# VachaLab/gorder

Measured on AMD Instinct MI355X. Metric: trajectory frames/sec, higher is better.
Workload: dtype f32

## Files before the change

### gorder_amd/abi.py

```python
from __future__ import annotations

import ctypes as C
import os
from dataclasses import dataclass, field
from typing import List, Optional, Sequence

import numpy as np

_HERE = os.path.dirname(os.path.abspath(__file__))
LIB_PATH = os.environ.get("GORDER_HIP_LIB") or os.path.join(_HERE, "libgorder_hip.so")

OK = 0
ERR_UNDEFINED_BOX = 1
ERR_NOT_ORTHOGONAL_BOX = 2
ERR_ZERO_BOX = 3
ERR_UNDEFINED_POSITION = 4
ERR_INVALID_GLOBAL_MEMBRANE_CENTER = 5
ERR_INVALID_LOCAL_MEMBRANE_CENTER = 6
ERR_INVALID_ARGUMENT = 100
ERR_DEVICE = 101
ERR_NO_DEVICE = 102
ERR_BOX_RANGE = 103
ERR_LEAFLETS_NOT_PRIMED = 104
ERR_OVERFLOW = 105
# ... 119 lines not shown
    flip: bool = False
    radius: float = 0.0
    membrane: Optional[np.ndarray] = None


@dataclass
class OrderMap:
    enabled: bool = False
    plane: int = 0
    span_x: Sequence[float] = (0.0, 0.0)
    span_y: Sequence[float] = (0.0, 0.0)
    bin: Sequence[float] = (0.1, 0.1)


GEOM_NONE, GEOM_CUBOID, GEOM_CYLINDER, GEOM_SPHERE = range(4)
GEOMREF_POINT, GEOMREF_BOX_CENTER, GEOMREF_GROUP = range(3)
_INF = float("inf")


@dataclass
class Geometry:
    kind: int = GEOM_NONE
    invert: bool = False
    reference: int = GEOMREF_POINT
    point: Sequence[float] = (0.0, 0.0, 0.0)
    group: Optional[np.ndarray] = None
    xdim: Sequence[float] = (-_INF, _INF)
    ydim: Sequence[float] = (-_INF, _INF)
    zdim: Sequence[float] = (-_INF, _INF)
    radius: float = 0.0
    span: Sequence[float] = (-_INF, _INF)
    orientation: int = 2
    structure_box: Sequence[float] = (0.0, 0.0, 0.0)


@dataclass
class DynamicNormal:
    enabled: bool = False
    radius: float = 2.0
    cloud: Optional[np.ndarray] = None


@dataclass
class Tables:
    n_atoms: int
    molecule_types: List[MolType]
    handle_pbc: bool = True
    normal: Sequence[float] = (0.0, 0.0, 1.0)
    leaflets: Leaflets = field(default_factory=Leaflets)
    ordermap: OrderMap = field(default_factory=OrderMap)
    timewise: bool = False
    device: int = 0
    flags: int = 0
    geometry: Geometry = field(default_factory=Geometry)
    dynamic_normal: DynamicNormal = field(default_factory=DynamicNormal)

    @property
    def n_acc(self) -> int:
        return sum(m.n_slots for m in self.molecule_types)

    @property
    def n_molecules_total(self) -> int:
        return sum(m.n_molecules for m in self.molecule_types)

    @property
    def n_samples_per_frame(self) -> int:
        return sum(m.n_slots * m.n_molecules for m in self.molecule_types)

    def as_ctypes(self):
        keep = []
        mts = (CMolType * max(1, len(self.molecule_types)))()
        for k, m in enumerate(self.molecule_types):
            c = mts[k]
            c.n_molecules = m.n_molecules
            b = _u32(m.bonds, (-1, m.n_molecules, 2)) if m.bonds is not None else None
            c.n_bond_types = 0 if b is None else b.shape[0]
            c.bonds = _ptr(b)
            ua = (CUaAtom * max(1, len(m.ua_atoms)))()
            for q, (kind, idx) in enumerate(m.ua_atoms):
                ia = _u32(idx, (m.n_molecules, 4))
                ua[q].kind = int(kind)
                ua[q].indices = _ptr(ia)
                keep.append(ia)
            c.n_ua_atoms = len(m.ua_atoms)
            c.ua_atoms = C.cast(ua, C.POINTER(CUaAtom))
            h = _u32(m.heads, (m.n_molecules,)) if m.heads is not None else None
            c.heads = _ptr(h)
            me = _u32(m.methyls, (m.n_molecules, -1)) if m.methyls is not None else None
            c.n_methyls = 0 if me is None else me.shape[1]
            c.methyls = _ptr(me)
            nh = _u32(m.normal_heads, (m.n_molecules,)) if m.normal_heads is not None else None
            c.normal_heads = _ptr(nh)
            keep += [b, ua, h, me, nh]
        t = CTables()
        t.n_atoms = self.n_atoms
        t.n_molecule_types = len(self.molecule_types)
        t.molecule_types = C.cast(mts, C.POINTER(CMolType))
        t.handle_pbc = 1 if self.handle_pbc else 0
        t.normal[:] = [float(x) for x in self.normal]
        lf = self.leaflets
        mem = _u32(lf.membrane) if lf.membrane is not None else None
        t.leaflets.method = lf.method
        t.leaflets.normal_dim = lf.normal_dim
        t.leaflets.frequency = lf.frequency
        t.leaflets.flip = 1 if lf.flip else 0
        t.leaflets.radius = lf.radius
        t.leaflets.n_membrane = 0 if mem is None else mem.size
        t.leaflets.membrane = _ptr(mem)
        om = self.ordermap
        t.ordermap.enabled = 1 if om.enabled else 0
        t.ordermap.plane = om.plane
        t.ordermap.span_x[:] = [float(x) for x in om.span_x]
        t.ordermap.span_y[:] = [float(x) for x in om.span_y]
        t.ordermap.bin[:] = [float(x) for x in om.bin]
        t.timewise = 1 if self.timewise else 0
        t.device = self.device
        t.flags = self.flags
        ge = self.geometry
        grp = _u32(ge.group) if ge.group is not None else None
        t.geometry.kind = ge.kind
        t.geometry.invert = 1 if ge.invert else 0
        t.geometry.reference = ge.reference
        t.geometry.point[:] = [float(x) for x in ge.point]
        t.geometry.n_group = 0 if grp is None else grp.size
        t.geometry.group = _ptr(grp)
        t.geometry.xdim[:] = [float(x) for x in ge.xdim]
        t.geometry.ydim[:] = [float(x) for x in ge.ydim]
        t.geometry.zdim[:] = [float(x) for x in ge.zdim]
        t.geometry.radius = ge.radius
        t.geometry.span[:] = [float(x) for x in ge.span]
        t.geometry.orientation = ge.orientation
        t.geometry.structure_box[:] = [float(x) for x in ge.structure_box]
        dn = self.dynamic_normal
        cloud = _u32(dn.cloud) if dn.cloud is not None else None
        t.dynamic_normal.enabled = 1 if dn.enabled else 0
        t.dynamic_normal.radius = dn.radius
        t.dynamic_normal.n_cloud = 0 if cloud is None else cloud.size
        t.dynamic_normal.cloud = _ptr(cloud)
        keep += [mts, mem, grp, cloud]
        return t, keep


_EXPORTS = [
    "gorder_hip_create", "gorder_hip_destroy", "gorder_hip_n_accumulators", "gorder_hip_ordermap_dims",
    "gorder_hip_set_stream", "gorder_hip_submit_device", "gorder_hip_submit_host",
    "gorder_hip_prime_leaflets", "gorder_hip_set_manual_leaflets", "gorder_hip_synchronize",
    "gorder_hip_finish", "gorder_hip_timewise", "gorder_hip_leaflets", "gorder_hip_leaflet_distances",
    "gorder_hip_normals", "gorder_hip_export_maps", "gorder_hip_set_normals",
    "gorder_hip_accumulators_device", "gorder_hip_bind_accumulators", "gorder_hip_last_error_index", "gorder_hip_last_error_frame", "gorder_hip_kernel_time_names",
    "gorder_hip_last_error_message", "gorder_hip_strerror", "gorder_hip_kernel_time", "gorder_hip_kernel_time_group", "gorder_hip_plan",
    "gorder_hip_plan_tables", "gorder_hip_selftest_arithmetic", "gorder_hip_selftest_trig", "gorder_hip_run_trajectory",
    "gorder_hip_comm_unique_id", "gorder_hip_comm_create", "gorder_hip_comm_destroy", "gorder_hip_allreduce",
    "gorder_hip_reset", "gorder_hip_xtc_decode", "gorder_hip_release_staging", "gorder_hip_speculation_stats", "gorder_hip_local_decide_stats",
    "gorder_hip_spherical_stats",
]

_lib = None


class GorderHipError(RuntimeError):
    def __init__(self, status: int, message: str = "", index: int = 0, frame: int = 0):
        self.status = status
        self.index = index
        self.frame = frame
        super().__init__(f"gorder_hip status {status}: {message}")


def load_library() -> C.CDLL:
    global _lib
    if _lib is not None:
        return _lib
    if not os.path.exists(LIB_PATH):
        raise GorderHipError(ERR_NO_DEVICE, f"{LIB_PATH} is missing: run `python -c 'import __graft_entry__ as g; "
                                            "g.build()'` (there is no CPU fallback)")
    try:
        import torch
        _rt = os.path.join(os.path.dirname(torch.__file__), "lib", "libamdhip64.so")
        if os.path.exists(_rt):
            C.CDLL(_rt, mode=C.RTLD_GLOBAL)
    except ImportError:
        pass
    lib = C.CDLL(LIB_PATH)
    vp, u32, u64, i32 = C.c_void_p, C.c_uint32, C.c_uint64, C.c_int
    lib.gorder_hip_create.argtypes = [C.POINTER(CTables), C.POINTER(vp)]
    lib.gorder_hip_destroy.argtypes = [vp]
    lib.gorder_hip_destroy.restype = None
    lib.gorder_hip_n_accumulators.argtypes = [vp]
    lib.gorder_hip_n_accumulators.restype = u32
    lib.gorder_hip_ordermap_dims.argtypes = [vp, C.POINTER(u32), C.POINTER(u32)]
    lib.gorder_hip_ordermap_dims.restype = u32
    lib.gorder_hip_set_stream.argtypes = [vp, vp]
    lib.gorder_hip_submit_device.argtypes = [vp, vp, vp, vp, u32]
    lib.gorder_hip_submit_host.argtypes = [vp, vp, vp, vp, u32]
    lib.gorder_hip_prime_leaflets.argtypes = [vp, vp, vp, u64]
    lib.gorder_hip_set_manual_leaflets.argtypes = [vp, vp, u64]
    lib.gorder_hip_synchronize.argtypes = [vp]
    lib.gorder_hip_finish.argtypes = [vp, vp, vp, vp, vp, C.POINTER(u64)]
    lib.gorder_hip_timewise.argtypes = [vp, vp, vp, u64]
    lib.gorder_hip_leaflets.argtypes = [vp, vp, C.POINTER(u64)]
    lib.gorder_hip_leaflet_distances.argtypes = [vp, vp]
    lib.gorder_hip_normals.argtypes = [vp, vp, vp]
    lib.gorder_hip_export_maps.argtypes = [vp, vp, vp, u64]
    lib.gorder_hip_set_normals.argtypes = [vp, vp, u32]
    lib.gorder_hip_accumulators_device.argtypes = [vp, C.POINTER(vp), C.POINTER(u64)]
    lib.gorder_hip_bind_accumulators.argtypes = [vp, vp, u64]
    lib.gorder_hip_last_error_index.argtypes = [vp]
    lib.gorder_hip_last_error_index.restype = u64
    lib.gorder_hip_kernel_time_names.argtypes = [vp]
    lib.gorder_hip_kernel_time_names.restype = C.c_char_p
    lib.gorder_hip_last_error_frame.argtypes = [vp]
    lib.gorder_hip_last_error_frame.restype = u64
    lib.gorder_hip_last_error_message.argtypes = [vp]
    lib.gorder_hip_last_error_message.restype = C.c_char_p
    lib.gorder_hip_strerror.argtypes = [i32]
    lib.gorder_hip_strerror.restype = C.c_char_p
    lib.gorder_hip_kernel_time.argtypes = [vp, C.POINTER(C.c_double), C.POINTER(u64), i32]
    lib.gorder_hip_kernel_time_group.argtypes = [vp, C.c_uint32, C.POINTER(C.c_char_p), C.POINTER(C.c_double), C.POINTER(u64)]
    lib.gorder_hip_plan.argtypes = [vp, C.POINTER(CPlan)]
    lib.gorder_hip_speculation_stats.argtypes = [vp, C.POINTER(C.c_uint64)]
    lib.gorder_hip_local_decide_stats.argtypes = [vp, C.POINTER(C.c_uint64)]
    lib.gorder_hip_spherical_stats.argtypes = [vp, C.POINTER(C.c_float)]
    lib.gorder_hip_plan_tables.argtypes = [C.POINTER(CTables), C.POINTER(CPlan), C.POINTER(i32)]
    lib.gorder_hip_selftest_arithmetic.argtypes = [i32, C.c_uint64, C.c_uint64, C.POINTER(C.c_uint64)]
    lib.gorder_hip_selftest_trig.argtypes = [i32, i32, C.c_uint32, C.c_uint32, C.c_uint32, C.c_void_p]
    lib.gorder_hip_run_trajectory.argtypes = [vp, C.POINTER(CTrajectory), C.POINTER(CTrajectoryStats)]
    lib.gorder_hip_comm_unique_id.argtypes = [vp]
    lib.gorder_hip_comm_create.argtypes = [vp, vp, i32, i32, C.POINTER(vp)]
    lib.gorder_hip_comm_destroy.argtypes = [vp]
    lib.gorder_hip_comm_destroy.restype = None
    lib.gorder_hip_allreduce.argtypes = [vp, vp]
    lib.gorder_hip_reset.argtypes = [vp]
    lib.gorder_hip_xtc_decode.argtypes = [vp, vp, u64, vp, u32, u32, vp, u32, vp, u32]
    lib.gorder_hip_release_staging.argtypes = [vp]
    lib.gorder_hip_release_staging.restype = None
    _lib = lib
    return lib


def selftest_trig(fn: str, first_bits: int, stride: int, n: int, device: int = 0) -> np.ndarray:
    lib = load_library()
    out = np.empty(n, dtype=np.float32)
    st = lib.gorder_hip_selftest_trig(device, {"acos": 0, "acos_cores": 1, "cos": 2, "sin": 3}[fn], first_bits, stride, n, out.ctypes.data)
    if st != 0:
        raise GorderHipError(st, "gorder_hip_selftest_trig")
    return out


def selftest_arithmetic(n: int = 1 << 26, seed: int = 1, device: int = 0):
    lib = load_library()
    out = (C.c_uint64 * 2)()
    st = lib.gorder_hip_selftest_arithmetic(device, n, seed, out)
    if st != 0:
        raise GorderHipError(st, lib.gorder_hip_strerror(st).decode())
    return int(out[0]), int(out[1])


def plan_tables(tables: Tables) -> dict:
    lib = load_library()
    ct, keep = tables.as_ctypes()
    plan, check = CPlan(), C.c_int(-1)
    st = lib.gorder_hip_plan_tables(C.byref(ct), C.byref(plan), C.byref(check))
    if st != OK:
        raise GorderHipError(st, lib.gorder_hip_strerror(st).decode())
    d = {name: getattr(plan, name) for name, _ in CPlan._fields_}
    d["selfcheck"] = check.value
    return d


@dataclass
class Results:
    sums: np.ndarray
    counts: np.ndarray
    n_frames: int
    map_sums: Optional[np.ndarray] = None
    map_counts: Optional[np.ndarray] = None

    def order_ticks(self, min_samples: int = 1) -> np.ndarray:
        n = self.counts.astype(np.int64)
        ok = n >= max(1, min_samples)
        q = np.full(self.sums.shape, np.iinfo(np.int64).min, dtype=np.int64)
        q[ok] = (np.abs(self.sums[ok]) // n[ok]) * np.sign(self.sums[ok])
        return q

    def order(self, min_samples: int = 1) -> np.ndarray:
        out = np.full(self.sums.shape, np.nan, dtype=np.float32)
        n = self.counts.astype(np.int64)
        ok = n >= max(1, min_samples)
        q = (np.abs(self.sums[ok]) // n[ok]) * np.sign(self.sums[ok])
        out[ok] = (q.astype(np.float64) / 1e6).astype(np.float32)
        return out


class HipEngine:

    def __init__(self, tables: Tables):
        self.lib = load_library()
        self.tables = tables
        ct, keep = tables.as_ctypes()
        self._h = C.c_void_p()
        st = self.lib.gorder_hip_create(C.byref(ct), C.byref(self._h))
        if st != OK:
            msg = self.lib.gorder_hip_strerror(st).decode()
            if self._h:
                msg += ": " + self.lib.gorder_hip_last_error_message(self._h).decode()
                self.lib.gorder_hip_destroy(self._h)
                self._h = C.c_void_p()
            raise GorderHipError(st, msg)
        self.n_acc = self.lib.gorder_hip_n_accumulators(self._h)
        self._keep = []

    def close(self):
        if getattr(self, "_h", None):
            self.lib.gorder_hip_destroy(self._h)
            self._h = C.c_void_p()

    def __del__(self):
        try:
            self.close()
        except Exception:
            pass

    def _check(self, st: int):
        if st != OK:
            msg = self.lib.gorder_hip_strerror(st).decode() + ": " + \
                self.lib.gorder_hip_last_error_message(self._h).decode()
            raise GorderHipError(st, msg, self.lib.gorder_hip_last_error_index(self._h),
                                 self.lib.gorder_hip_last_error_frame(self._h))

    def set_stream(self, stream_ptr: int):
        self._check(self.lib.gorder_hip_set_stream(self._h, C.c_void_p(stream_ptr)))

    def use_torch_stream(self):
        import torch
        self.set_stream(torch.cuda.current_stream().cuda_stream)

    @staticmethod
    def _frame_index(frame_index, n_frames):
        if frame_index is None:
            frame_index = np.arange(n_frames, dtype=np.uint64)
        fi = np.ascontiguousarray(frame_index, dtype=np.uint64)
        assert fi.shape == (n_frames,)
        return fi

    def submit_device(self, xyz, box, frame_index=None):
        assert xyz.is_cuda and xyz.is_contiguous() and xyz.dtype.is_floating_point and xyz.element_size() == 4
        n_frames = xyz.shape[0]
        assert xyz.shape[1] == self.tables.n_atoms and xyz.shape[2] == 3
        fi = self._frame_index(frame_index, n_frames)
        bp = None
        if box is not None:
            assert box.is_cuda and box.is_contiguous() and box.numel() == 9 * n_frames
            bp = C.c_void_p(box.data_ptr())
        self._check(self.lib.gorder_hip_submit_device(self._h, C.c_void_p(xyz.data_ptr()), bp,
                                                      fi.ctypes.data_as(C.c_void_p), n_frames))

    def submit_host(self, xyz: np.ndarray, box: Optional[np.ndarray], frame_index=None):
        xyz = np.ascontiguousarray(xyz, dtype=np.float32)
        n_frames = xyz.shape[0]
        assert xyz.shape[1:] == (self.tables.n_atoms, 3)
        fi = self._frame_index(frame_index, n_frames)
        bp = None
        if box is not None:
            box = np.ascontiguousarray(box, dtype=np.float32).reshape(n_frames, 9)
            bp = box.ctypes.data_as(C.c_void_p)
        self._check(self.lib.gorder_hip_submit_host(self._h, xyz.ctypes.data_as(C.c_void_p), bp,
                                                    fi.ctypes.data_as(C.c_void_p), n_frames))

    def run_trajectory(self, paths, group=None, begin: float = 0.0, end: float = -1.0, step: int = 1, threads: int = 0,
                       batch_frames: int = 0, first_frame_index: int = 0, device_decode: bool = False,
                       shard=None) -> dict:
        arr = (C.c_char_p * len(paths))(*[p.encode() for p in paths])
        grp = None if group is None else np.ascontiguousarray(group, dtype=np.uint32)
        t = CTrajectory()
# ... 4 lines not shown
        t.begin_ps, t.end_ps, t.step = begin, end, step
        t.n_threads, t.batch_frames, t.first_frame_index = threads, batch_frames, first_frame_index
        t.device_decode = 1 if device_decode else 0
        if shard is not None:
            t.shard_index, t.shard_count = shard
        stats = CTrajectoryStats()
        self._check(self.lib.gorder_hip_run_trajectory(self._h, C.byref(t), C.byref(stats)))
        return {name: getattr(stats, name) for name, _ in CTrajectoryStats._fields_}

    def xtc_decode(self, d_blob: int, blob_bytes: int, d_frames: int, n_frames: int, n_atoms_file: int, d_slot_of: int,
                   n_stop: int, d_xyz: int, n_atoms_out: int):
        self._check(self.lib.gorder_hip_xtc_decode(self._h, d_blob, blob_bytes, d_frames, n_frames, n_atoms_file,
                                                   d_slot_of or None, n_stop, d_xyz, n_atoms_out))

    def release_staging(self):
        self.lib.gorder_hip_release_staging(self._h)

    def reset(self):
        self._check(self.lib.gorder_hip_reset(self._h))

    @staticmethod
    def comm_unique_id() -> bytes:
        lib = load_library()
        buf = (C.c_uint8 * 128)()
        st = lib.gorder_hip_comm_unique_id(buf)
        if st != OK:
            raise GorderHipError(st, "ncclGetUniqueId failed (is RCCL loadable?)")
        return bytes(buf)

    def comm_create(self, unique_id: bytes, n_ranks: int, rank: int):
        assert len(unique_id) == 128
        buf = (C.c_uint8 * 128).from_buffer_copy(unique_id)
        comm = C.c_void_p()
        self._check(self.lib.gorder_hip_comm_create(self._h, buf, n_ranks, rank, C.byref(comm)))
        return comm

    def comm_destroy(self, comm):
        self.lib.gorder_hip_comm_destroy(comm)

    def allreduce(self, comm):
        self._check(self.lib.gorder_hip_allreduce(self._h, comm))

    def prime_leaflets_device(self, xyz, box, frame_index: int):
        bp = C.c_void_p(box.data_ptr()) if box is not None else None
        self._check(self.lib.gorder_hip_prime_leaflets(self._h, C.c_void_p(xyz.data_ptr()), bp, frame_index))

    def set_manual_leaflets(self, flags: np.ndarray, frame_index: int = 0):
        flags = np.ascontiguousarray(flags, dtype=np.uint8)
        assert flags.size == self.tables.n_molecules_total
        self._check(self.lib.gorder_hip_set_manual_leaflets(self._h, flags.ctypes.data_as(C.c_void_p), frame_index))

    def synchronize(self):
        self._check(self.lib.gorder_hip_synchronize(self._h))

    def ordermap_dims(self):
        nx, ny = C.c_uint32(), C.c_uint32()
        nt = self.lib.gorder_hip_ordermap_dims(self._h, C.byref(nx), C.byref(ny))
        return (int(nx.value), int(ny.value)) if nt else (0, 0)

    def finish(self) -> Results:
        n = self.n_acc
        sums = np.zeros((3, n), dtype=np.int64)
        counts = np.zeros((3, n), dtype=np.uint64)
        nx, ny = C.c_uint32(), C.c_uint32()
        nt = self.lib.gorder_hip_ordermap_dims(self._h, C.byref(nx), C.byref(ny))
        ms = mc = None
        msp = mcp = None
        if nt:
            ms = np.zeros((3, n, nx.value, ny.value), dtype=np.int64)
            mc = np.zeros((3, n, nx.value, ny.value), dtype=np.uint64)
            msp, mcp = ms.ctypes.data_as(C.c_void_p), mc.ctypes.data_as(C.c_void_p)
        nf = C.c_uint64()
        self._check(self.lib.gorder_hip_finish(self._h, sums.ctypes.data_as(C.c_void_p),
                                               counts.ctypes.data_as(C.c_void_p), msp, mcp, C.byref(nf)))
        return Results(sums, counts, int(nf.value), ms, mc)

    def timewise(self, n_frames: int):
        n = self.n_acc
        s = np.zeros((n_frames, 3, n), dtype=np.int64)
        c = np.zeros((n_frames, 3, n), dtype=np.uint64)
        self._check(self.lib.gorder_hip_timewise(self._h, s.ctypes.data_as(C.c_void_p),
                                                 c.ctypes.data_as(C.c_void_p), n_frames))
        return s, c

    def leaflets(self):
        flags = np.zeros(self.tables.n_molecules_total, dtype=np.uint8)
        fr = C.c_uint64()
        self._check(self.lib.gorder_hip_leaflets(self._h, flags.ctypes.data_as(C.c_void_p), C.byref(fr)))
        return flags, int(fr.value)

    def leaflet_distances(self) -> np.ndarray:
        d = np.zeros(self.tables.n_molecules_total, dtype=np.float32)
        self._check(self.lib.gorder_hip_leaflet_distances(self._h, d.ctypes.data_as(C.c_void_p)))
        return d

    def set_normals(self, normals: np.ndarray):
        n = np.ascontiguousarray(normals, dtype=np.float32)
        assert n.ndim == 3 and n.shape[1:] == (self.tables.n_molecules_total, 3)
        self._check(self.lib.gorder_hip_set_normals(self._h, n.ctypes.data_as(C.c_void_p), n.shape[0]))

    def normals(self):
        n = np.zeros((self.tables.n_molecules_total, 3), dtype=np.float32)
        k = np.zeros(self.tables.n_molecules_total, dtype=np.uint32)
        self._check(self.lib.gorder_hip_normals(self._h, n.ctypes.data_as(C.c_void_p), k.ctypes.data_as(C.c_void_p)))
        return n, k

    def accumulator_words(self) -> int:
        p, n = C.c_void_p(), C.c_uint64()
        self._check(self.lib.gorder_hip_accumulators_device(self._h, C.byref(p), C.byref(n)))
        return int(n.value)

    def flush(self):
        self.accumulator_words()

    def bind_accumulators(self, tensor):
        assert tensor.is_cuda and tensor.is_contiguous() and tensor.element_size() == 8
        self._keep.append(tensor)
        self._check(self.lib.gorder_hip_bind_accumulators(self._h, C.c_void_p(tensor.data_ptr()), tensor.numel()))

    def export_maps(self, sums, counts):
        for t in (sums, counts):
            assert t.is_cuda and t.is_contiguous() and t.element_size() == 8
        assert sums.numel() == counts.numel()
        self._check(self.lib.gorder_hip_export_maps(self._h, C.c_void_p(sums.data_ptr()), C.c_void_p(counts.data_ptr()),
                                                     sums.numel()))

    def kernel_time(self, reset: bool = False):
        ms, n = C.c_double(), C.c_uint64()
        self._check(self.lib.gorder_hip_kernel_time(self._h, C.byref(ms), C.byref(n), 1 if reset else 0))
        return ms.value, int(n.value)

    def kernel_names(self) -> str:
        return self.lib.gorder_hip_kernel_time_names(self._h).decode()

    def kernel_groups(self):
        out, k = [], 0
        while True:
            name, ms, n = C.c_char_p(), C.c_double(), C.c_uint64()
            if self.lib.gorder_hip_kernel_time_group(self._h, k, C.byref(name), C.byref(ms), C.byref(n)) != 0:
                return out
            out.append((name.value.decode(), ms.value, int(n.value)))
            k += 1

    def speculation_stats(self) -> dict:
        out = (C.c_uint64 * 4)()
        self._check(self.lib.gorder_hip_speculation_stats(self._h, out))
        return {"batches": int(out[0]), "moved": int(out[1]), "exact_frames": int(out[2]), "enabled": bool(out[3])}

    def local_decide_stats(self) -> dict:
        out = (C.c_uint64 * 4)()
        self._check(self.lib.gorder_hip_local_decide_stats(self._h, out))
        return {"submits": int(out[0]), "paused": int(out[1]), "open_frames": int(out[2]), "frames": int(out[3])}

    def spherical_stats(self) -> dict:
        out = (C.c_float * 12)()
        self._check(self.lib.gorder_hip_spherical_stats(self._h, out))
        v = np.array(out[:], dtype=np.float32)
        return {"centre": v[0:3].copy(), "weight_a": v[3], "mean_a": v[4], "var_a": v[5], "mean_b": v[6], "var_b": v[7],
                "avg_log_likelihood": v[8], "iterations": int(v[9]), "n_outer": int(v[10])}

    def plan(self) -> dict:
        p = CPlan()
        self._check(self.lib.gorder_hip_plan(self._h, C.byref(p)))
        return {name: getattr(p, name) for name, _ in CPlan._fields_}
```

### gorder_amd/csrc/gorder_hip.hip

```cpp
#include <hip/hip_runtime.h>

#include <dlfcn.h>

#include <cmath>
#include <cstdio>
#include <cstdlib>
#include <cstring>
#include <mutex>
#include <new>
#include <string>
#include <deque>
#include <vector>

#include "../../include/gorder_hip.h"
#include "gm_math.h"
#include "plan.h"

#pragma clang fp contract(off)

using gorder::DirectItem;
using gorder::Item;
using gorder::kBlock;
using gorder::Plan;
using gorder::Tile;

#include "kernels_common.h"
#include "kernels_bonds.h"
#include "kernels_extras.h"
#include "kernels_leaflets.h"
#include "kernels_normals.h"
#include "kernels_xtc.h"


struct gorder_hip_handle {
    void *traj_cache = nullptr;
    void (*traj_cache_free)(gorder_hip_handle *) = nullptr;
    Plan plan;
    gorder_tables_t tables{};
    int device = 0;
    hipStream_t own_stream = nullptr;
    hipStream_t stream = nullptr;
    Tile *d_tiles = nullptr;
    Item *d_items = nullptr;
    uint32_t *d_tile_slots = nullptr;
    DirectItem *d_direct = nullptr;
    Tile *d_ua_tiles = nullptr;
    gorder::UaItem *d_ua_items = nullptr;
    uint32_t *d_ua_tile_slots = nullptr;
    uint32_t map_nx = 0, map_ny = 0;
    unsigned long long *d_map_sums = nullptr, *d_map_cnts = nullptr;
    unsigned long long *d_map_packed = nullptr;
    unsigned long long *d_map_rec = nullptr;
    size_t map_rec_cap = 0;
    gorder::MapRun *d_ua_runs = nullptr, *d_runs = nullptr;
    uint32_t *d_ua_run_begin = nullptr, *d_run_begin = nullptr;
    Item *d_items_by_slot = nullptr;
    uint32_t *d_ua_item_run = nullptr, *d_item_run = nullptr;
    uint4 *d_lgrid = nullptr;
    LocalRowPre *d_lrowpre = nullptr;
    LocalEdge *d_ledge = nullptr;
    float4 *d_lfinfo = nullptr;
    static constexpr uint32_t kDecidePause = 16;
    uint32_t *d_lsummary = nullptr, *h_lsummary = nullptr;
    hipEvent_t lsummary_written = nullptr;
    bool lsummary_pending = false;
    uint32_t decide_pause = 0;
    uint64_t decide_submits = 0, decide_paused_submits = 0;
    uint32_t *d_lneed = nullptr;
    uint2 *d_ltodo = nullptr;
    size_t map_lds_bytes = 0;
    bool map_staged = false;
    uint64_t map_pending = 0;
    uint64_t map_fold_limit = kMapFoldLimit;
    uint32_t map_max_mol = 1;
    unsigned long long *d_tw_sums = nullptr, *d_tw_cnts = nullptr;
    uint64_t tw_cap = 0;
    ExtraArgs extra{};
    uint32_t *d_geom_group = nullptr;
    float *d_shapes = nullptr;
    float *d_inv_box = nullptr;
    size_t inv_box_cap = 0;
    uint32_t dyn_slab = 4, local_slab = 4;
    bool local_halo = false;
    size_t local_rec_stride = 0;
    XtcCheckpoint *d_xtc_cp = nullptr;
    size_t xtc_cp_cap = 0;
    bool dyn = false;
    uint32_t *d_dyn_cloud = nullptr, *d_dyn_heads = nullptr;
    uint32_t *d_dyn_cell_of = nullptr, *d_dyn_count = nullptr;
    float *d_dyn_rec = nullptr;
    float4 *d_dyn_normals = nullptr;
    DynCov *d_dyn_cov = nullptr;
    size_t dyn_normals_cap = 0;
    std::vector<float> last_normals;
    std::vector<float> manual_normals;
    uint32_t manual_frames = 0;
    bool manual_active = false;
    size_t shapes_cap = 0;
    uint32_t *d_err = nullptr;
    unsigned long long *d_acc = nullptr;
    unsigned long long *d_rep = nullptr;
    uint32_t n_rep = 32;
    bool rep_dirty = false;
    bool acc_external = false;
    size_t acc_words = 0;
    uint32_t *d_heads = nullptr, *d_membrane = nullptr, *d_methyl_begin = nullptr, *d_methyl_atoms = nullptr;
    uint8_t *d_aflags = nullptr;
    size_t aflags_rows = 0;
    float *d_adist = nullptr;
    float *d_sph_spill = nullptr, *d_sph_stats = nullptr;
    uint32_t sph_spill = 0, sph_slab = 1u << 20, sph_threads = 1024;
    uint32_t *d_lcell_of = nullptr, *d_lcell_count = nullptr, *d_lcell_fill = nullptr;
    float *d_ltrig = nullptr;
    uint32_t *d_arow = nullptr, *d_aframes = nullptr;
    std::vector<uint32_t> up_arow, up_aframes;
    const uint32_t *up_arow_at = nullptr, *up_aframes_at = nullptr;
    size_t arow_cap = 0, aframes_cap = 0;
    bool have_assignment = false;
    uint64_t assignment_frame = 0;
    bool spec_enabled = false;
    bool spec_now = false;
    uint2 *d_own = nullptr;
    float4 *d_mom = nullptr;
    size_t mom_cap = 0;
    float *d_head_z = nullptr;
    size_t head_z_cap = 0;
    uint32_t *d_own_head_begin = nullptr;
    uint2 *d_own_heads = nullptr;
    float *d_spec_center = nullptr;
    uint8_t *d_spec_ok = nullptr;
    size_t spec_frames_cap = 0;
    uint32_t *d_spec_counters = nullptr;
    static constexpr uint32_t kSpecRing = 8;
    uint32_t *h_spec_counters = nullptr;
    hipEvent_t spec_counters_copied[kSpecRing] = {};
    uint64_t spec_ring_frames[kSpecRing] = {};
    uint32_t *d_spec_mol_begin = nullptr;
    SpecSample *d_spec_samples = nullptr;
    uint64_t spec_batches = 0, spec_fixed = 0, spec_exact_frames = 0;
    float *d_stage_xyz[2] = {nullptr, nullptr}, *d_stage_box[2] = {nullptr, nullptr};
    size_t stage_xyz_cap[2] = {0, 0}, stage_box_cap[2] = {0, 0};
    hipEvent_t stage_copied[2] = {nullptr, nullptr}, stage_computed[2] = {nullptr, nullptr};
    bool stage_used[2] = {false, false};
    int stage_next = 0;
    hipStream_t copy_stream = nullptr;
    float n2 = 1.0f, n2sq = 1.0f;
    int axis = -1;
    int frames_per_stage = kFramesPerStage;
    bool membrane_is_frame = false;
    bool use_gather = false;
    uint32_t wg_capacity = 256u * 6u;
    uint32_t wg_target = 0;
    uint32_t lw = 0;
    size_t lds_bytes = 0;
    uint64_t n_frames = 0;
    uint64_t err_index = 0;
    std::string err_msg;
    static constexpr uint32_t kTimingEvents = 1024;
    struct TimingSeg { uint32_t label, ev_a, ev_b; };
    bool timing_on = false;
    hipEvent_t timing_ev[kTimingEvents] = {};
    uint32_t timing_next_ev = 0;
    int timing_open_label = -1;
    uint32_t timing_open_ev = 0;
    std::deque<TimingSeg> timing_pending;
    std::vector<std::string> timing_labels;
    std::vector<double> timing_label_ms;
    std::vector<uint64_t> timing_label_n;
    uint64_t timing_launches = 0;
    std::string timed_kernels;
    std::vector<uint32_t> host_heads, host_dyn_heads;
    uint32_t *d_mol_slot0 = nullptr;
    uint64_t err_frame = 0;
    struct BatchLog { uint64_t ordinal, first, stride; std::vector<uint64_t> list; };
    static constexpr size_t kBatchLog = 4096;
    std::deque<BatchLog> batch_log;
    uint64_t n_submits = 0;
    const unsigned long long *decoder_key = nullptr;
};

namespace {

int fail(gorder_hip_handle *h, int status, const std::string &msg) {
    if (h) h->err_msg = msg;
    return status;
}

#define HIP_TRY(h, expr)                                                                    \
    do {                                                                                    \
        hipError_t e_ = (expr);                                                             \
        if (e_ != hipSuccess)                                                               \
            return fail(h, GORDER_ERR_DEVICE, std::string(#expr) + ": " + hipGetErrorString(e_)); \
    } while (0)

template <typename T>
int upload(gorder_hip_handle *h, T **dst, const std::vector<T> &src) {
    *dst = nullptr;
    if (src.empty()) return GORDER_OK;
    HIP_TRY(h, hipMalloc((void **)dst, src.size() * sizeof(T)));
    HIP_TRY(h, hipMemcpy(*dst, src.data(), src.size() * sizeof(T), hipMemcpyHostToDevice));
    return GORDER_OK;
}

template <typename T>
int ensure(gorder_hip_handle *h, T **buf, size_t *cap, size_t need) {
    if (need <= *cap) return GORDER_OK;
    if (*buf) HIP_TRY(h, hipFree(*buf));
    *buf = nullptr;
    *cap = 0;
    const size_t n = need + need / 2;
    HIP_TRY(h, hipMalloc((void **)buf, n * sizeof(T)));
    *cap = n;
    return GORDER_OK;
}

bool should_assign(uint32_t frequency, uint64_t frame) {
// ... 773 lines not shown
        if (e != hipSuccess || per_cu < 1) per_cu = 4;
        h->wg_capacity = (uint32_t)n_cu * (uint32_t)per_cu;
    }

    const gorder_dynamic_normal_t &dn = t->dynamic_normal;
    if (dn.enabled) {
        if (!(dn.radius > 0.0f)) return fail(h, GORDER_ERR_INVALID_ARGUMENT, "dynamic normals need a positive radius");
        if (!dn.cloud || dn.n_cloud == 0) return fail(h, GORDER_ERR_INVALID_ARGUMENT, "dynamic normals need the NormalHeads group");
        if (!p.direct.empty()) return fail(h, GORDER_ERR_INVALID_ARGUMENT, "dynamic normals: a bond spans more than the LDS window");
        std::vector<uint32_t> cloud(dn.cloud, dn.cloud + dn.n_cloud), nheads;
        for (uint32_t a : cloud)
            if (a >= t->n_atoms) return fail(h, GORDER_ERR_INVALID_ARGUMENT, "NormalHeads index out of range");
        for (uint32_t m = 0; m < t->n_molecule_types; m++) {
            const gorder_moltype_t &mt = t->molecule_types[m];
            if (!mt.normal_heads) return fail(h, GORDER_ERR_INVALID_ARGUMENT, "dynamic normals need normal_heads[] per molecule type");
            for (uint32_t k = 0; k < mt.n_molecules; k++) {
                if (mt.normal_heads[k] >= t->n_atoms) return fail(h, GORDER_ERR_INVALID_ARGUMENT, "normal head index out of range");
                nheads.push_back(mt.normal_heads[k]);
            }
        }
        if ((st = upload(h, &h->d_dyn_cloud, cloud)) != GORDER_OK) return st;
        if ((st = upload(h, &h->d_dyn_heads, nheads)) != GORDER_OK) return st;
        h->host_dyn_heads = nheads;
        const size_t nm = dn.n_cloud, ncell = (size_t)kLocalMaxCells1D * kLocalMaxCells1D;
        const size_t sl = h->dyn_slab = local_slab_frames(nm);
        for (const void *fn : {reinterpret_cast<const void *>(k_local_build<2>), reinterpret_cast<const void *>(k_local_build<5>),
                               reinterpret_cast<const void *>(k_local_build<kLocalBuildTrips>)})
            HIP_TRY(h, hipFuncSetAttribute(fn, hipFuncAttributeMaxDynamicSharedMemorySize, (int)kLocalBuildLds));
        HIP_TRY(h, hipMalloc((void **)&h->d_dyn_cell_of, sl * nm * sizeof(uint32_t)));
        HIP_TRY(h, hipMalloc((void **)&h->d_dyn_rec, sl * nm * 4 * sizeof(float)));
        HIP_TRY(h, hipMalloc((void **)&h->d_dyn_count, sl * (2 * ncell + 1) * sizeof(uint32_t)));
        HIP_TRY(h, hipMalloc((void **)&h->d_dyn_cov, sl * (size_t)(p.n_mol_total ? p.n_mol_total : 1) * sizeof(DynCov)));
        h->dyn = true;
    }

    const gorder_leaflets_t &lf = t->leaflets;
    if (lf.method != GORDER_LEAFLETS_NONE) {
        if (lf.method > GORDER_LEAFLETS_SPHERICAL) return fail(h, GORDER_ERR_INVALID_ARGUMENT, "leaflets.method");
        if (lf.method != GORDER_LEAFLETS_SPHERICAL && lf.normal_dim > 2) return fail(h, GORDER_ERR_INVALID_ARGUMENT, "leaflets.normal_dim");
        std::vector<uint32_t> heads, mb(1, 0), ma;
        for (uint32_t m = 0; m < t->n_molecule_types; m++) {
            const gorder_moltype_t &mt = t->molecule_types[m];
            if (lf.method != GORDER_LEAFLETS_MANUAL && !mt.heads)
                return fail(h, GORDER_ERR_INVALID_ARGUMENT, "leaflets need heads[] per molecule type");
            if (lf.method == GORDER_LEAFLETS_INDIVIDUAL && (!mt.methyls || mt.n_methyls == 0))
                return fail(h, GORDER_ERR_INVALID_ARGUMENT, "individual leaflets need methyls[]");
            for (uint32_t k = 0; k < mt.n_molecules; k++) {
                const uint32_t hd = mt.heads ? mt.heads[k] : 0;
                if (hd >= t->n_atoms) return fail(h, GORDER_ERR_INVALID_ARGUMENT, "head index out of range");
                heads.push_back(hd);
                if (lf.method == GORDER_LEAFLETS_INDIVIDUAL)
                    for (uint32_t q = 0; q < mt.n_methyls; q++) {
                        const uint32_t a = mt.methyls[(size_t)k * mt.n_methyls + q];
                        if (a >= t->n_atoms) return fail(h, GORDER_ERR_INVALID_ARGUMENT, "methyl index out of range");
                        ma.push_back(a);
                    }
                mb.push_back((uint32_t)ma.size());
            }
        }
        if ((st = upload(h, &h->d_heads, heads)) != GORDER_OK) return st;
        h->host_heads = heads;
        if (lf.method == GORDER_LEAFLETS_LOCAL) {
            std::vector<uint32_t> ms;
            for (uint32_t m = 0; m < t->n_molecule_types; m++) ms.insert(ms.end(), t->molecule_types[m].n_molecules, p.slot0[m]);
            if ((st = upload(h, &h->d_mol_slot0, ms)) != GORDER_OK) return st;
        }
        if ((st = upload(h, &h->d_methyl_begin, mb)) != GORDER_OK) return st;
        if ((st = upload(h, &h->d_methyl_atoms, ma)) != GORDER_OK) return st;
        if (lf.method == GORDER_LEAFLETS_LOCAL && !(lf.radius > 0.0f))
            return fail(h, GORDER_ERR_INVALID_ARGUMENT, "local leaflets need a positive radius");
        if (lf.method == GORDER_LEAFLETS_GLOBAL || lf.method == GORDER_LEAFLETS_LOCAL) {
            if (!lf.membrane || lf.n_membrane == 0)
                return fail(h, GORDER_ERR_INVALID_ARGUMENT, "global/local leaflets need the membrane group");
            std::vector<uint32_t> mem(lf.membrane, lf.membrane + lf.n_membrane);
            for (uint32_t a : mem)
                if (a >= t->n_atoms) return fail(h, GORDER_ERR_INVALID_ARGUMENT, "membrane index out of range");
            if ((st = upload(h, &h->d_membrane, mem)) != GORDER_OK) return st;
            h->membrane_is_frame = lf.n_membrane == t->n_atoms && !env_flag("GORDER_HIP_LEAFLETS_GENERIC");
            for (uint32_t i = 0; i < lf.n_membrane && h->membrane_is_frame; i++) h->membrane_is_frame = mem[i] == i;
        }
        if (lf.method == GORDER_LEAFLETS_SPHERICAL) {
            if (!lf.membrane || lf.n_membrane < 2)
                return fail(h, GORDER_ERR_INVALID_ARGUMENT, "leaflets.n_membrane: spherical clustering needs at least two group atoms");
            std::vector<uint32_t> grp(lf.membrane, lf.membrane + lf.n_membrane);
            std::vector<int32_t> slot_of(t->n_atoms, -1);
            for (uint32_t i = 0; i < lf.n_membrane; i++) {
                if (grp[i] >= t->n_atoms) return fail(h, GORDER_ERR_INVALID_ARGUMENT, "leaflets.membrane: index out of range");
                if (slot_of[grp[i]] < 0) slot_of[grp[i]] = (int32_t)i;
            }
            for (uint32_t hd : heads)
                if (slot_of[hd] < 0)
                    return fail(h, GORDER_ERR_INVALID_ARGUMENT, "molecule_types[].heads: a head is not a member of leaflets.membrane");
            if ((st = upload(h, &h->d_membrane, grp)) != GORDER_OK) return st;
            h->sph_threads = lf.n_membrane <= 256u * (uint32_t)kSphKeep ? 256u : 1024u;
            const uint32_t resident = h->sph_threads * (uint32_t)kSphKeep;
            h->sph_spill = lf.n_membrane > resident ? lf.n_membrane - resident : 0u;
            if (h->sph_spill) {
                h->sph_slab = (uint32_t)std::min<size_t>(std::max<size_t>(((size_t)64 << 20) / (h->sph_spill * sizeof(float)), 1), 4096);
                HIP_TRY(h, hipMalloc((void **)&h->d_sph_spill, (size_t)h->sph_slab * h->sph_spill * sizeof(float)));
            }
            HIP_TRY(h, hipMalloc((void **)&h->d_sph_stats, 12 * sizeof(float)));
            HIP_TRY(h, hipMemset(h->d_sph_stats, 0, 12 * sizeof(float)));
        }
        if (lf.method == GORDER_LEAFLETS_GLOBAL && p.spec_ok && !env_flag("GORDER_HIP_NO_SPECULATE")) {
            std::vector<uint2> own(p.tiles.size());
            for (size_t i = 0; i < own.size(); i++) own[i] = make_uint2(p.own[2 * i], p.own[2 * i + 1]);
            if ((st = upload(h, &h->d_own, own)) != GORDER_OK) return st;
            std::vector<std::vector<SpecSample>> per_mol(p.n_mol_total);
            for (const Tile &tile : p.tiles)
                for (uint32_t q = 0; q < tile.n_items; q++) {
                    const Item &it = p.items[tile.item0 + q];
                    per_mol[it.mol].push_back({tile.atom0 + it.li, tile.atom0 + it.lj, p.tile_slots[tile.slot0 + it.lslot]});
                }
            std::vector<uint32_t> mbeg(1, 0);
            std::vector<SpecSample> all;
            for (const auto &v : per_mol) { all.insert(all.end(), v.begin(), v.end()); mbeg.push_back((uint32_t)all.size()); }
            if ((st = upload(h, &h->d_spec_mol_begin, mbeg)) != GORDER_OK) return st;
            if ((st = upload(h, &h->d_spec_samples, all)) != GORDER_OK) return st;
            std::vector<uint2> oh(p.own_heads.size() / 2);
            for (size_t i = 0; i < oh.size(); i++) oh[i] = make_uint2(p.own_heads[2 * i], p.own_heads[2 * i + 1]);
            if ((st = upload(h, &h->d_own_head_begin, p.own_head_begin)) != GORDER_OK) return st;
            if ((st = upload(h, &h->d_own_heads, oh)) != GORDER_OK) return st;
            HIP_TRY(h, hipMalloc((void **)&h->d_spec_counters, 4 * sizeof(uint32_t)));
            HIP_TRY(h, hipMemset(h->d_spec_counters, 0, 4 * sizeof(uint32_t)));
            HIP_TRY(h, hipHostMalloc((void **)&h->h_spec_counters, 2 * gorder_hip_handle::kSpecRing * sizeof(uint32_t)));
            for (hipEvent_t &ev : h->spec_counters_copied) HIP_TRY(h, hipEventCreateWithFlags(&ev, hipEventDisableTiming));
            h->spec_enabled = true;
        }
        if (lf.method == GORDER_LEAFLETS_LOCAL) {
            const size_t nm = lf.n_membrane, ncell = (size_t)kLocalMaxCells1D * kLocalMaxCells1D;
            const size_t sl = h->local_slab = local_slab_frames(nm);
            for (const void *fn : {reinterpret_cast<const void *>(k_local_build<2>), reinterpret_cast<const void *>(k_local_build<5>),
                                   reinterpret_cast<const void *>(k_local_build<kLocalBuildTrips>)})
                HIP_TRY(h, hipFuncSetAttribute(fn, hipFuncAttributeMaxDynamicSharedMemorySize, (int)kLocalBuildLds));
            h->local_halo = t->handle_pbc && !env_flag("GORDER_HIP_LOCAL_ATOMS_ONLY");
            h->local_rec_stride = (h->local_halo ? 2u : 1u) * nm;
            HIP_TRY(h, hipMalloc((void **)&h->d_lcell_of, sl * nm * sizeof(uint32_t)));
            HIP_TRY(h, hipMalloc((void **)&h->d_ltrig, sl * h->local_rec_stride * sizeof(LocalRec)));
            HIP_TRY(h, hipMalloc((void **)&h->d_lcell_count, sl * (ncell + 1) * sizeof(uint32_t)));
            HIP_TRY(h, hipMalloc((void **)&h->d_lcell_fill, sl * ncell * sizeof(uint32_t)));
            HIP_TRY(h, hipMalloc((void **)&h->d_lgrid, sl * sizeof(uint4)));
            if (h->local_halo) {
                HIP_TRY(h, hipMalloc((void **)&h->d_lrowpre, sl * (size_t)kLocalMaxCells1D * (kLocalMaxCells1D + 1u) * sizeof(LocalRowPre)));
                HIP_TRY(h, hipMalloc((void **)&h->d_ledge, sl * (size_t)kLocalMaxCells1D * (kLocalMaxCells1D + 1u) * sizeof(LocalEdge)));
                HIP_TRY(h, hipMalloc((void **)&h->d_lfinfo, sl * sizeof(float4)));
                HIP_TRY(h, hipMalloc((void **)&h->d_lneed, (sl + 1) * sizeof(uint32_t)));
                HIP_TRY(h, hipMalloc((void **)&h->d_lsummary, 2 * sizeof(uint32_t)));
                HIP_TRY(h, hipMemset(h->d_lsummary, 0, 2 * sizeof(uint32_t)));
                HIP_TRY(h, hipHostMalloc((void **)&h->h_lsummary, 2 * sizeof(uint32_t)));
                h->h_lsummary[0] = h->h_lsummary[1] = 0u;
                HIP_TRY(h, hipEventCreateWithFlags(&h->lsummary_written, hipEventDisableTiming));
                HIP_TRY(h, hipFuncSetAttribute(reinterpret_cast<const void *>(k_local_decide), hipFuncAttributeMaxDynamicSharedMemorySize,
                                               (int)kDecideLds));
                HIP_TRY(h, hipFuncSetAttribute(reinterpret_cast<const void *>(k_local_sums), hipFuncAttributeMaxDynamicSharedMemorySize,
                                               (int)kSumsLds));
                HIP_TRY(h, hipMalloc((void **)&h->d_ltodo, (1 + sl * (size_t)(p.n_mol_total ? p.n_mol_total : 1)) * sizeof(uint2)));
            }
        }
        HIP_TRY(h, hipMalloc((void **)&h->d_adist, sizeof(float) * (p.n_mol_total ? p.n_mol_total : 1)));
    }
    HIP_TRY(h, hipDeviceSynchronize());
    return GORDER_OK;
}

void gorder_hip_destroy(gorder_hip_handle *h) {
    if (!h) return;
    (void)hipSetDevice(h->device);
    if (h->stream) (void)hipStreamSynchronize(h->stream);
    if (h->traj_cache_free) h->traj_cache_free(h);
    for (hipEvent_t ev : h->timing_ev)
        if (ev) (void)hipEventDestroy(ev);
    (void)hipFree(h->d_mol_slot0);
    (void)hipFree(h->d_tiles); (void)hipFree(h->d_items); (void)hipFree(h->d_tile_slots);
    (void)hipFree(h->d_direct); (void)hipFree(h->d_err); (void)hipFree(h->d_xtc_cp);
    (void)hipFree(h->d_ua_tiles); (void)hipFree(h->d_ua_items); (void)hipFree(h->d_ua_tile_slots);
    (void)hipFree(h->d_map_sums); (void)hipFree(h->d_map_cnts); (void)hipFree(h->d_map_packed); (void)hipFree(h->d_tw_sums); (void)hipFree(h->d_tw_cnts);
    (void)hipFree(h->d_geom_group); (void)hipFree(h->d_shapes); (void)hipFree(h->d_inv_box);
    (void)hipFree(h->d_map_rec); (void)hipFree(h->d_ua_runs); (void)hipFree(h->d_ua_run_begin);
    (void)hipFree(h->d_runs); (void)hipFree(h->d_run_begin); (void)hipFree(h->d_items_by_slot);
    (void)hipFree(h->d_ua_item_run); (void)hipFree(h->d_item_run); (void)hipFree(h->d_lgrid); (void)hipFree(h->d_lrowpre); (void)hipFree(h->d_ledge);
    (void)hipFree(h->d_own); (void)hipFree(h->d_mom); (void)hipFree(h->d_head_z); (void)hipFree(h->d_own_head_begin); (void)hipFree(h->d_own_heads); (void)hipFree(h->d_spec_center); (void)hipFree(h->d_spec_ok);
    (void)hipFree(h->d_spec_counters); (void)hipFree(h->d_spec_mol_begin); (void)hipFree(h->d_spec_samples);
    if (h->h_spec_counters) (void)hipHostFree(h->h_spec_counters);
    for (hipEvent_t ev : h->spec_counters_copied) if (ev) (void)hipEventDestroy(ev); (void)hipFree(h->d_lfinfo); (void)hipFree(h->d_ltodo); (void)hipFree(h->d_lneed);
    (void)hipFree(h->d_lsummary); if (h->h_lsummary) (void)hipHostFree(h->h_lsummary); if (h->lsummary_written) (void)hipEventDestroy(h->lsummary_written);
    (void)hipFree(h->d_dyn_cloud); (void)hipFree(h->d_dyn_heads); (void)hipFree(h->d_dyn_cell_of); (void)hipFree(h->d_dyn_count);
    (void)hipFree(h->d_dyn_rec); (void)hipFree(h->d_dyn_normals); (void)hipFree(h->d_dyn_cov);
    if (!h->acc_external) (void)hipFree(h->d_acc);
    (void)hipFree(h->d_rep);
    (void)hipFree(h->d_heads); (void)hipFree(h->d_membrane); (void)hipFree(h->d_methyl_begin);
    (void)hipFree(h->d_methyl_atoms); (void)hipFree(h->d_aflags); (void)hipFree(h->d_adist);
    (void)hipFree(h->d_sph_spill); (void)hipFree(h->d_sph_stats);
    (void)hipFree(h->d_arow); (void)hipFree(h->d_aframes);
    (void)hipFree(h->d_lcell_of); (void)hipFree(h->d_lcell_count); (void)hipFree(h->d_lcell_fill);
    (void)hipFree(h->d_ltrig);
    for (int k = 0; k < 2; k++) {
        (void)hipFree(h->d_stage_xyz[k]); (void)hipFree(h->d_stage_box[k]);
        if (h->stage_copied[k]) (void)hipEventDestroy(h->stage_copied[k]);
        if (h->stage_computed[k]) (void)hipEventDestroy(h->stage_computed[k]);
    }
    if (h->copy_stream) (void)hipStreamDestroy(h->copy_stream);
    if (h->own_stream) (void)hipStreamDestroy(h->own_stream);
    delete h;
}

uint32_t gorder_hip_n_accumulators(const gorder_hip_handle *h) { return h ? h->plan.n_acc : 0; }
uint32_t gorder_hip_ordermap_dims(const gorder_hip_handle *h, uint32_t *nx, uint32_t *ny) {
    if (nx) *nx = h ? h->map_nx : 0;
    if (ny) *ny = h ? h->map_ny : 0;
    return h ? h->map_nx * h->map_ny : 0;
}

int gorder_hip_set_stream(gorder_hip_handle *h, void *hip_stream) {
    if (!h) return GORDER_ERR_INVALID_ARGUMENT;
    HIP_TRY(h, hipSetDevice(h->device));
    HIP_TRY(h, hipStreamSynchronize(h->stream));
    h->stream = hip_stream ? (hipStream_t)hip_stream : h->own_stream;
    return GORDER_OK;
}

static void spec_poll(gorder_hip_handle *h, bool wait);
int gorder_hip_speculation_stats(gorder_hip_handle *h, uint64_t out[4]) {
    if (!h || !out) return GORDER_ERR_INVALID_ARGUMENT;
    HIP_TRY(h, hipSetDevice(h->device));
    HIP_TRY(h, hipStreamSynchronize(h->stream));
    spec_poll(h, true);
    out[0] = h->spec_batches; out[1] = h->spec_fixed; out[2] = h->spec_exact_frames; out[3] = h->spec_enabled ? 1 : 0;
    return GORDER_OK;
}

int gorder_hip_local_decide_stats(gorder_hip_handle *h, uint64_t out[4]) {
    if (!h || !out) return GORDER_ERR_INVALID_ARGUMENT;
    HIP_TRY(h, hipSetDevice(h->device));
    HIP_TRY(h, hipStreamSynchronize(h->stream));
    out[0] = h->decide_submits; out[1] = h->decide_paused_submits;
    out[2] = h->h_lsummary ? h->h_lsummary[0] : 0; out[3] = h->h_lsummary ? h->h_lsummary[1] : 0;
    return GORDER_OK;
}

int gorder_hip_plan(const gorder_hip_handle *h, gorder_hip_plan_t *plan) {
    if (!h || !plan) return GORDER_ERR_INVALID_ARGUMENT;
    plan->n_tiles = (uint32_t)h->plan.tiles.size();
    plan->block_threads = kBlock;
    plan->max_window_atoms = h->plan.max_window;
    plan->n_direct_items = (uint32_t)h->plan.direct.size();
    plan->frames_per_stage = (uint32_t)h->frames_per_stage;
    plan->lds_bytes = (uint32_t)h->lds_bytes;
    plan->map_staged = h->map_staged ? 1u : 0u;
    plan->map_lds_bytes = (uint32_t)h->map_lds_bytes;
    plan->leaflets_one_read = h->plan.spec_ok ? 1u : 0u;
    return GORDER_OK;
}

static void spec_poll(gorder_hip_handle *h, bool wait) {
    for (uint32_t i = 0; i < gorder_hip_handle::kSpecRing; i++) {
        if (!h->spec_ring_frames[i]) continue;
        if (wait) (void)hipEventSynchronize(h->spec_counters_copied[i]);
        else if (hipEventQuery(h->spec_counters_copied[i]) != hipSuccess) continue;
        const uint32_t moved = h->h_spec_counters[2 * i], exact = h->h_spec_counters[2 * i + 1];
        h->spec_fixed += moved;
        h->spec_exact_frames += exact;
        if ((uint64_t)exact * 8u > h->spec_ring_frames[i] ||
            (uint64_t)moved * 16u > h->spec_ring_frames[i] * h->plan.n_mol_total)
            h->spec_enabled = false;
        h->spec_ring_frames[i] = 0;
    }
}

static int run_leaflets(gorder_hip_handle *h, const float *d_xyz, const float *d_box,
                        const std::vector<uint32_t> &aframes, uint32_t row0, const uint8_t *skip = nullptr) {
    if (aframes.empty()) return GORDER_OK;
    int st;
    const size_t cap_before = h->aframes_cap;
    if ((st = ensure(h, &h->d_aframes, &h->aframes_cap, aframes.size())) != GORDER_OK) return st;
    if (h->aframes_cap != cap_before) h->up_aframes_at = nullptr;
    if (h->up_aframes_at != h->d_aframes || h->up_aframes != aframes) {
        HIP_TRY(h, hipMemcpyAsync(h->d_aframes, aframes.data(), aframes.size() * sizeof(uint32_t),
                                  hipMemcpyHostToDevice, h->stream));
        h->up_aframes = aframes;
        h->up_aframes_at = h->d_aframes;
    }
    const gorder_leaflets_t &lf = h->tables.leaflets;
    LeafletArgs la{};
    la.xyz = d_xyz; la.box9 = d_box; la.n_atoms = h->plan.n_atoms;
    la.aframes = h->d_aframes; la.row0 = row0; la.aflags = h->d_aflags; la.adist = h->d_adist;
    la.n_mol_total = h->plan.n_mol_total; la.heads = h->d_heads;
    la.membrane = h->d_membrane; la.n_membrane = lf.n_membrane;
    la.methyl_begin = h->d_methyl_begin; la.methyl_atoms = h->d_methyl_atoms;
    la.dim = lf.normal_dim; la.flip = lf.flip ? 1 : 0; la.pbc = h->tables.handle_pbc ? 1 : 0;
    la.err = h->d_err;
    la.skip = skip;
    la.n_assign = (uint32_t)aframes.size();
    if (lf.method == GORDER_LEAFLETS_GLOBAL) {
        const dim3 g(skip ? std::min<uint32_t>((uint32_t)aframes.size(), 512u) : (uint32_t)aframes.size()), b(1024);
        TIMING_MARK(h, h->membrane_is_frame ? "k_leaflets_global_contig" : "k_leaflets_global");
        if (h->membrane_is_frame) {
            if (skip) hipLaunchKernelGGL(k_leaflets_global_contig<true>, g, dim3(256), 0, h->stream, la);
            else hipLaunchKernelGGL(k_leaflets_global_contig<false>, g, dim3(256), 0, h->stream, la);
        } else {
            if (skip) hipLaunchKernelGGL(k_leaflets_global<true>, g, b, 0, h->stream, la);
            else hipLaunchKernelGGL(k_leaflets_global<false>, g, b, 0, h->stream, la);
        }
    } else if (lf.method == GORDER_LEAFLETS_INDIVIDUAL) {
        TIMING_MARK(h, "k_leaflets_individual");
        size_t done = 0;
        while (done < aframes.size()) {
            const uint32_t ny = (uint32_t)std::min<size_t>(aframes.size() - done, 65535);
            LeafletArgs lb = la;
            lb.aframes = h->d_aframes + done;
            lb.row0 = row0 + (uint32_t)done;
            if (done + ny < aframes.size()) lb.adist = nullptr;
            hipLaunchKernelGGL(k_leaflets_individual, dim3((la.n_mol_total + 255) / 256, ny), dim3(256), 0,
                               h->stream, lb);
            done += ny;
        }
    } else if (lf.method == GORDER_LEAFLETS_SPHERICAL) {
        TIMING_MARK(h, "k_leaflets_spherical");
        SphArgs sa{};
        sa.xyz = d_xyz; sa.box9 = d_box; sa.n_atoms = h->plan.n_atoms;
        sa.aflags = h->d_aflags; sa.n_mol_total = h->plan.n_mol_total; sa.heads = h->d_heads;
        sa.group = h->d_membrane; sa.n_group = lf.n_membrane;
        sa.flip = lf.flip ? 1 : 0; sa.pbc = h->tables.handle_pbc ? 1 : 0;
        sa.spill = h->d_sph_spill; sa.n_spill = h->sph_spill; sa.err = h->d_err;
        for (size_t done = 0; done < aframes.size(); done += h->sph_slab) {
            const uint32_t ns = (uint32_t)std::min<size_t>(aframes.size() - done, h->sph_slab);
            const bool last = done + ns == aframes.size();
            sa.aframes = h->d_aframes + done;
            sa.row0 = row0 + (uint32_t)done;
            sa.n_assign = ns;
            sa.adist = last ? h->d_adist : nullptr;
            sa.stats = last ? h->d_sph_stats : nullptr;
            if (h->sph_threads == 256u) hipLaunchKernelGGL(k_leaflets_spherical<256>, dim3(ns), dim3(256), 0, h->stream, sa);
            else hipLaunchKernelGGL(k_leaflets_spherical<1024>, dim3(ns), dim3(1024), 0, h->stream, sa);
        }
    } else if (lf.method == GORDER_LEAFLETS_LOCAL) {
        const size_t ncell = (size_t)kLocalMaxCells1D * kLocalMaxCells1D;
        LocalArgs lo{};
        lo.xyz = d_xyz; lo.box9 = d_box; lo.n_atoms = h->plan.n_atoms;
        lo.aflags = h->d_aflags; lo.adist = h->d_adist; lo.n_mol_total = h->plan.n_mol_total;
        lo.heads = h->d_heads; lo.mol_slot0 = h->d_mol_slot0; lo.n_membrane = lf.n_membrane;
        lo.membrane = h->membrane_is_frame ? nullptr : h->d_membrane;
        lo.dim = lf.normal_dim; lo.flip = lf.flip ? 1 : 0; lo.pbc = h->tables.handle_pbc ? 1 : 0;
        lo.radius = lf.radius;
        lo.radius_thr = local_radius_threshold(lf.radius);
        lo.cell_of = h->d_lcell_of; lo.trig = h->d_ltrig; lo.cell_count = h->d_lcell_count;
        lo.cell_fill = h->d_lcell_fill; lo.err = h->d_err;
        lo.grid = h->d_lgrid;
        lo.halo = h->local_halo ? 1 : 0;
        lo.prune = env_flag("GORDER_HIP_LOCAL_NO_PRUNE") ? 0 : (env_flag("GORDER_HIP_LOCAL_DECIDE_NOTHING") ? 2 : 1);
        lo.rec_stride = (uint32_t)h->local_rec_stride;
        lo.rowpre = h->d_lrowpre;
        lo.edge = h->d_ledge;
        lo.finfo = h->d_lfinfo;
        lo.todo = h->d_ltodo;
        bool decide = lo.halo && lo.prune && lo.n_mol_total && !env_flag("GORDER_HIP_LOCAL_NO_DECIDE");
        if (decide) {
            if (h->lsummary_pending) {
                if (hipEventQuery(h->lsummary_written) == hipSuccess) {
                    h->lsummary_pending = false;
                    if (2u * h->h_lsummary[0] > h->h_lsummary[1]) h->decide_pause = gorder_hip_handle::kDecidePause;
                } else {
                    (void)hipGetLastError();
                }
            }
            if (h->decide_pause) { h->decide_pause--; h->decide_paused_submits++; decide = false; }
            else h->decide_submits++;
        }
        lo.need = decide ? h->d_lneed : nullptr;
        lo.sums = decide && lf.n_membrane <= kLocalBuildMax && !env_flag("GORDER_HIP_LOCAL_THREE_KERNELS") &&
                  !env_flag("GORDER_HIP_LOCAL_NO_SUMS") ? 1 : 0;
        const bool report = decide && !h->lsummary_pending;
        lo.summary = report ? h->d_lsummary : nullptr;
        for (size_t done = 0; done < aframes.size(); done += h->local_slab) {
            const uint32_t ns = (uint32_t)std::min<size_t>(aframes.size() - done, h->local_slab);
            lo.aframes = h->d_aframes + done;
            lo.n_slab = ns;
            lo.row0 = row0 + (uint32_t)done;
            lo.write_dist_frame = (done + ns == aframes.size()) ? (int)ns - 1 : -1;
            lo.summary_host = report && done + ns == aframes.size() ? h->h_lsummary : nullptr;
            if (lf.n_membrane > kLocalBuildMax || env_flag("GORDER_HIP_LOCAL_THREE_KERNELS"))
                HIP_TRY(h, hipMemsetAsync(h->d_lcell_fill, 0, ns * ncell * sizeof(uint32_t), h->stream));
            if (lo.sums) {
                HIP_TRY(h, hipMemsetAsync(h->d_lneed, 0, (ns + 1) * sizeof(uint32_t), h->stream));
                TIMING_MARK(h, "k_local_sums");
                hipLaunchKernelGGL(k_local_sums, dim3(ns), dim3(1024), kSumsLds, h->stream, lo);
                TIMING_MARK(h, "k_local_decide");
                hipLaunchKernelGGL(k_local_decide, dim3(ns), dim3(1024), kDecideLds, h->stream, lo);
            }
            const int cst = launch_cell_list(h, lo, ns, lf.n_membrane, h->d_lcell_count, ns * (ncell + 1) * sizeof(uint32_t));
            if (cst != GORDER_OK) return cst;
            if (lo.halo) {
                TIMING_MARK(h, "k_local_rowprefix");
                hipLaunchKernelGGL(k_local_rowprefix, dim3(kLocalMaxCells1D / 4u, ns), dim3(256), 0, h->stream, lo);
                lo.rows_groups = (lo.n_mol_total + 15u) / 16u;
                if (lo.need && !lo.sums) {
                    TIMING_MARK(h, "k_local_decide");
                    hipLaunchKernelGGL(k_local_decide, dim3(ns), dim3(1024), kDecideLds, h->stream, lo);
                }
                TIMING_MARK(h, "k_local_flags_rows");
                if (lo.need) hipLaunchKernelGGL(k_local_flags_rows_open, dim3(lo.rows_groups * 8u * kRowsSlots), dim3(256), 0, h->stream, lo);
                else hipLaunchKernelGGL(k_local_flags_rows, dim3(lo.rows_groups * ((ns + 7u) / 8u * 8u)), dim3(256), 0, h->stream, lo);
                TIMING_MARK(h, "k_local_flags_todo");
                hipLaunchKernelGGL(k_local_flags_todo, dim3(512), dim3(256), 0, h->stream, lo);
            } else {
                TIMING_MARK(h, "k_local_flags");
                hipLaunchKernelGGL(k_local_flags, dim3((lo.n_mol_total + 3) / 4, ns), dim3(256), 0, h->stream, lo);
            }
        }
        if (report && !aframes.empty()) {
            HIP_TRY(h, hipEventRecord(h->lsummary_written, h->stream));
            h->lsummary_pending = true;
        }
    }
    HIP_TRY(h, hipGetLastError());
    return GORDER_OK;
}

int gorder_hip_submit_device(gorder_hip_handle *h, const float *d_xyz, const float *d_box,
                             const uint64_t *frame_index, uint32_t n_frames) {
    if (!h || !d_xyz || !frame_index) return GORDER_ERR_INVALID_ARGUMENT;
    const bool pbc = h->tables.handle_pbc != 0;
    if (pbc && !d_box) return fail(h, GORDER_ERR_INVALID_ARGUMENT, "box required when handle_pbc = 1");
    if (((uintptr_t)d_xyz & 15u) != 0) return fail(h, GORDER_ERR_INVALID_ARGUMENT, "d_xyz must be 16-byte aligned");
    if (n_frames == 0) return GORDER_OK;
    HIP_TRY(h, hipSetDevice(h->device));
    const Plan &p = h->plan;
    const gorder_leaflets_t &lf = h->tables.leaflets;
    int st;
    if ((h->n_frames + n_frames) > (uint64_t)(9223372036854775807ll / 1000000ll) / h->map_max_mol)
        return fail(h, GORDER_ERR_OVERFLOW, "order accumulators could overflow i64 (frames x molecules >= 2^63 / 1e6)");

    const bool leaflets = lf.method != GORDER_LEAFLETS_NONE;
    size_t n_new_rows = 0;
    bool spec = false;
    std::vector<uint32_t> spec_aframes;
    if (h->manual_frames) {
        if (h->manual_frames != n_frames) return fail(h, GORDER_ERR_INVALID_ARGUMENT, "gorder_hip_set_normals: frame count differs from the batch");
        if (!p.direct.empty()) return fail(h, GORDER_ERR_INVALID_ARGUMENT, "manual normals: a bond spans more than the LDS window");
    }
    auto abort_batch = [&](int status) {
        hipLaunchKernelGGL(k_batch_abort, dim3(1), dim3(1), 0, h->stream, h->d_err);
        (void)hipGetLastError();
        (void)timing_mark(h, nullptr);
        return status;
    };
    if (leaflets) {
        std::vector<uint32_t> arow(n_frames), aframes;
        uint32_t cur = 0;
        bool have = h->have_assignment;
        uint64_t last_assign_frame = h->assignment_frame;
        for (uint32_t f = 0; f < n_frames; f++) {
            if (lf.method != GORDER_LEAFLETS_MANUAL && should_assign(lf.frequency, frame_index[f])) {
                aframes.push_back(f);
                cur = (uint32_t)aframes.size();
                have = true;
                last_assign_frame = frame_index[f];
            }
            if (!have) return fail(h, GORDER_ERR_LEAFLETS_NOT_PRIMED, "no leaflet assignment for the first frame");
            arow[f] = cur;
        }
        const bool tw_tiled = h->extra.tw && !(h->tables.flags & GORDER_FLAG_TRIG_ACOS_COS) && h->d_item_run &&
                              h->frames_per_stage == (int)kRecFrames && !env_flag("GORDER_HIP_TW_GATHER");
        spec = h->spec_enabled && lf.method == GORDER_LEAFLETS_GLOBAL && h->have_assignment && aframes.size() == n_frames &&
               !h->extra.maps && (!h->extra.tw || tw_tiled) && !h->extra.geom_kind && !h->dyn && !h->manual_frames &&
               !h->use_gather && !p.tiles.empty();
        if (spec) {
            spec_poll(h, false);
            const uint32_t slot = (uint32_t)(h->spec_batches % gorder_hip_handle::kSpecRing);
            if (h->spec_ring_frames[slot]) (void)hipEventSynchronize(h->spec_counters_copied[slot]), spec_poll(h, false);
            spec = h->spec_enabled;
        }
        if (spec) std::fill(arow.begin(), arow.end(), 0u);
        const size_t rows = aframes.size() + 1;
        if (rows > h->aflags_rows) {
            uint8_t *nb = nullptr;
            const size_t nrows = rows + rows / 4;
            HIP_TRY(h, hipMalloc((void **)&nb, nrows * (size_t)p.n_mol_total));
            if (h->d_aflags) {
                HIP_TRY(h, hipMemcpyAsync(nb, h->d_aflags, p.n_mol_total, hipMemcpyDeviceToDevice, h->stream));
                HIP_TRY(h, hipStreamSynchronize(h->stream));
                HIP_TRY(h, hipFree(h->d_aflags));
            }
            h->d_aflags = nb;
            h->aflags_rows = nrows;
        }
        const size_t cap_before = h->arow_cap;
        if ((st = ensure(h, &h->d_arow, &h->arow_cap, n_frames)) != GORDER_OK) return st;
        if (h->arow_cap != cap_before) h->up_arow_at = nullptr;
        if (h->up_arow_at != h->d_arow || h->up_arow != arow) {
            HIP_TRY(h, hipMemcpyAsync(h->d_arow, arow.data(), n_frames * sizeof(uint32_t), hipMemcpyHostToDevice,
                                      h->stream));
            h->up_arow = arow;
            h->up_arow_at = h->d_arow;
        }
        if (spec) spec_aframes = aframes;
        else if ((st = run_leaflets(h, d_xyz, d_box, aframes, 1)) != GORDER_OK) return abort_batch(st);
        h->have_assignment = true;
        h->assignment_frame = last_assign_frame;
        n_new_rows = spec ? 0 : aframes.size();
    }
    if (h->extra.tw && h->n_frames + n_frames > h->tw_cap) {
        const size_t row = 3 * (size_t)p.n_acc;
        const uint64_t ncap = (h->n_frames + n_frames) * 2;
        unsigned long long *ns = nullptr, *nc = nullptr;
        HIP_TRY(h, hipMalloc((void **)&ns, ncap * row * sizeof(unsigned long long)));
        HIP_TRY(h, hipMalloc((void **)&nc, ncap * row * sizeof(unsigned long long)));
        HIP_TRY(h, hipMemsetAsync(ns, 0, ncap * row * sizeof(unsigned long long), h->stream));
        HIP_TRY(h, hipMemsetAsync(nc, 0, ncap * row * sizeof(unsigned long long), h->stream));
        if (h->d_tw_sums) {
            HIP_TRY(h, hipMemcpyAsync(ns, h->d_tw_sums, h->n_frames * row * sizeof(unsigned long long), hipMemcpyDeviceToDevice, h->stream));
            HIP_TRY(h, hipMemcpyAsync(nc, h->d_tw_cnts, h->n_frames * row * sizeof(unsigned long long), hipMemcpyDeviceToDevice, h->stream));
            HIP_TRY(h, hipStreamSynchronize(h->stream));
            HIP_TRY(h, hipFree(h->d_tw_sums));
            HIP_TRY(h, hipFree(h->d_tw_cnts));
        }
        h->d_tw_sums = ns; h->d_tw_cnts = nc; h->tw_cap = ncap;
    }
    FrameArgs a{};
    a.xyz = d_xyz; a.box9 = d_box; a.n_atoms = p.n_atoms; a.n_frames = n_frames;
    a.pbc = pbc ? 1 : 0;
    a.nx = h->tables.normal[0]; a.ny = h->tables.normal[1]; a.nz = h->tables.normal[2]; a.n2 = h->n2; a.n2sq = h->n2sq;
    a.leaflets = leaflets ? 1 : 0; a.aflags = h->d_aflags; a.arow = h->d_arow; a.n_mol_total = p.n_mol_total;
    a.acc = h->d_acc; a.rep = h->d_rep; a.n_rep = h->n_rep; a.n_acc = p.n_acc; a.err = h->d_err;
    h->manual_active = false;
    if (h->manual_frames) {
        const size_t n4 = (size_t)n_frames * p.n_mol_total;
        if ((st = ensure(h, &h->d_dyn_normals, &h->dyn_normals_cap, n4)) != GORDER_OK) return abort_batch(st);
        if (hipStreamSynchronize(h->stream) != hipSuccess ||
            hipMemcpy(h->d_dyn_normals, h->manual_normals.data(), n4 * 4 * sizeof(float), hipMemcpyHostToDevice) != hipSuccess)
            return abort_batch(fail(h, GORDER_ERR_DEVICE, "manual normals: copy to the device failed"));
        h->manual_active = true;
        h->manual_frames = 0;
    }
    const uint32_t n_tiles_all = (uint32_t)p.tiles.size();
    if (spec) {
        if ((st = ensure(h, &h->d_mom, &h->mom_cap, (size_t)n_frames * n_tiles_all)) != GORDER_OK) return abort_batch(st);
        if ((st = ensure(h, &h->d_head_z, &h->head_z_cap, (size_t)n_frames * p.n_mol_total)) != GORDER_OK) return abort_batch(st);
        a.own = h->d_own; a.mom = h->d_mom; a.mom_dim = (int)lf.normal_dim;
// ... 188 lines not shown
    h->manual_normals.resize(4 * n);
    for (size_t i = 0; i < n; i++) {
        h->manual_normals[4 * i + 0] = normals[3 * i + 0];
        h->manual_normals[4 * i + 1] = normals[3 * i + 1];
        h->manual_normals[4 * i + 2] = normals[3 * i + 2];
        h->manual_normals[4 * i + 3] = 3.0f;
    }
    h->manual_frames = n_frames;
    return GORDER_OK;
}

int gorder_hip_normals(gorder_hip_handle *h, float *normals, uint32_t *n_points) {
    if (!h || !h->dyn) return GORDER_ERR_INVALID_ARGUMENT;
    const int st = gorder_hip_synchronize(h);
    if (st != GORDER_OK) return st;
    const uint32_t n_mol = h->plan.n_mol_total;
    if (h->last_normals.size() < 4 * (size_t)n_mol) return fail(h, GORDER_ERR_INVALID_ARGUMENT, "no frame submitted yet");
    for (uint32_t m = 0; m < n_mol; m++) {
        if (normals) for (int d = 0; d < 3; d++) normals[3 * (size_t)m + d] = h->last_normals[4 * (size_t)m + d];
        if (n_points) n_points[m] = (uint32_t)h->last_normals[4 * (size_t)m + 3];
    }
    return GORDER_OK;
}

int gorder_hip_timewise(gorder_hip_handle *h, int64_t *tw_sums, uint64_t *tw_counts, uint64_t capacity_frames) {
    if (!h || !h->extra.tw || !tw_sums || !tw_counts) return GORDER_ERR_INVALID_ARGUMENT;
    if (capacity_frames < h->n_frames) return GORDER_ERR_INVALID_ARGUMENT;
    const int st = gorder_hip_synchronize(h);
    if (st != GORDER_OK) return st;
    const size_t n = h->n_frames * 3 * (size_t)h->plan.n_acc;
    if (n) {
        HIP_TRY(h, hipMemcpy(tw_sums, h->d_tw_sums, n * sizeof(int64_t), hipMemcpyDeviceToHost));
        HIP_TRY(h, hipMemcpy(tw_counts, h->d_tw_cnts, n * sizeof(uint64_t), hipMemcpyDeviceToHost));
        if (h->tables.leaflets.method != GORDER_LEAFLETS_NONE) {
            const size_t na = h->plan.n_acc;
            for (uint64_t f = 0; f < h->n_frames; f++) {
                int64_t *s = tw_sums + f * 3 * na;
                uint64_t *c = tw_counts + f * 3 * na;
                for (size_t k = 0; k < na; k++) { s[2 * na + k] = s[k] - s[na + k]; c[2 * na + k] = c[k] - c[na + k]; }
            }
        }
    }
    return GORDER_OK;
}

int gorder_hip_leaflets(gorder_hip_handle *h, uint8_t *flags, uint64_t *assignment_frame) {
    if (!h) return GORDER_ERR_INVALID_ARGUMENT;
    if (!h->have_assignment) return GORDER_ERR_LEAFLETS_NOT_PRIMED;
    const int st = gorder_hip_synchronize(h);
    if (st != GORDER_OK) return st;
    if (flags) HIP_TRY(h, hipMemcpy(flags, h->d_aflags, h->plan.n_mol_total, hipMemcpyDeviceToHost));
    if (assignment_frame) *assignment_frame = h->assignment_frame;
    return GORDER_OK;
}

int gorder_hip_leaflet_distances(gorder_hip_handle *h, float *dist) {
    if (!h || !dist || !h->d_adist) return GORDER_ERR_INVALID_ARGUMENT;
    const int st = gorder_hip_synchronize(h);
    if (st != GORDER_OK) return st;
    HIP_TRY(h, hipMemcpy(dist, h->d_adist, sizeof(float) * h->plan.n_mol_total, hipMemcpyDeviceToHost));
    return GORDER_OK;
}

int gorder_hip_spherical_stats(gorder_hip_handle *h, float out[12]) {
    if (!h || !out || h->tables.leaflets.method != GORDER_LEAFLETS_SPHERICAL || !h->d_sph_stats) return GORDER_ERR_INVALID_ARGUMENT;
    if (!h->have_assignment) return fail(h, GORDER_ERR_INVALID_ARGUMENT, "gorder_hip_spherical_stats: no assignment frame yet");
    const int st = gorder_hip_synchronize(h);
    if (st != GORDER_OK) return st;
    HIP_TRY(h, hipMemcpy(out, h->d_sph_stats, 12 * sizeof(float), hipMemcpyDeviceToHost));
    return GORDER_OK;
}

int gorder_hip_accumulators_device(gorder_hip_handle *h, void **d_ptr, uint64_t *n_u64) {
    if (!h || !d_ptr || !n_u64) return GORDER_ERR_INVALID_ARGUMENT;
    HIP_TRY(h, hipSetDevice(h->device));
    {
        const int st = fold_replicas(h);
        if (st != GORDER_OK) return st;
    }
    *d_ptr = h->d_acc;
    *n_u64 = h->acc_words;
    return GORDER_OK;
}

int gorder_hip_export_maps(gorder_hip_handle *h, void *d_sums, void *d_counts, uint64_t n_u64) {
    if (!h || !h->extra.maps || !d_sums || !d_counts) return GORDER_ERR_INVALID_ARGUMENT;
    const uint64_t n = 3ull * h->plan.n_acc * h->map_nx * h->map_ny;
    if (n_u64 < n) return GORDER_ERR_INVALID_ARGUMENT;
    HIP_TRY(h, hipSetDevice(h->device));
    const int st = fold_maps(h);
    if (st != GORDER_OK) return st;
    HIP_TRY(h, hipMemcpyAsync(d_sums, h->d_map_sums, n * sizeof(unsigned long long), hipMemcpyDeviceToDevice, h->stream));
    HIP_TRY(h, hipMemcpyAsync(d_counts, h->d_map_cnts, n * sizeof(unsigned long long), hipMemcpyDeviceToDevice, h->stream));
    HIP_TRY(h, hipStreamSynchronize(h->stream));
    return check_device_error(h);
}

int gorder_hip_bind_accumulators(gorder_hip_handle *h, void *d_ptr, uint64_t n_u64) {
    if (!h || !d_ptr || n_u64 < h->acc_words || ((uintptr_t)d_ptr & 7u)) return GORDER_ERR_INVALID_ARGUMENT;
    HIP_TRY(h, hipSetDevice(h->device));
    {
        const int st = fold_replicas(h);
        if (st != GORDER_OK) return st;
    }
    HIP_TRY(h, hipMemcpyAsync(d_ptr, h->d_acc, h->acc_words * sizeof(unsigned long long), hipMemcpyDeviceToDevice, h->stream));
    HIP_TRY(h, hipStreamSynchronize(h->stream));
    if (!h->acc_external) HIP_TRY(h, hipFree(h->d_acc));
    h->d_acc = (unsigned long long *)d_ptr;
    h->acc_external = true;
    return GORDER_OK;
}

int gorder_hip_reset(gorder_hip_handle *h) {
    if (!h) return GORDER_ERR_INVALID_ARGUMENT;
    HIP_TRY(h, hipSetDevice(h->device));
    const Plan &p = h->plan;
    HIP_TRY(h, hipMemsetAsync(h->d_acc, 0, h->acc_words * sizeof(unsigned long long), h->stream));
    if (h->d_rep) HIP_TRY(h, hipMemsetAsync(h->d_rep, 0, (size_t)h->n_rep * 4u * p.n_acc * sizeof(unsigned long long), h->stream));
    h->rep_dirty = false;
    if (h->extra.maps) {
        const size_t nmap = 3 * (size_t)p.n_acc * h->map_nx * h->map_ny;
        const size_t npk = (h->tables.leaflets.method != GORDER_LEAFLETS_NONE ? 2 : 1) * (nmap / 3);
        HIP_TRY(h, hipMemsetAsync(h->d_map_sums, 0, nmap * sizeof(unsigned long long), h->stream));
        HIP_TRY(h, hipMemsetAsync(h->d_map_cnts, 0, nmap * sizeof(unsigned long long), h->stream));
        HIP_TRY(h, hipMemsetAsync(h->d_map_packed, 0, npk * sizeof(unsigned long long), h->stream));
        h->map_pending = 0;
    }
    if (h->d_tw_sums) {
        const size_t n = h->tw_cap * 3 * (size_t)p.n_acc * sizeof(unsigned long long);
        HIP_TRY(h, hipMemsetAsync(h->d_tw_sums, 0, n, h->stream));
        HIP_TRY(h, hipMemsetAsync(h->d_tw_cnts, 0, n, h->stream));
    }
    HIP_TRY(h, hipMemsetAsync(h->d_err, 0xff, kErrWords * sizeof(uint32_t), h->stream));
    h->batch_log.clear();
    h->n_frames = 0;
    h->have_assignment = false;
    h->assignment_frame = 0;
    h->manual_frames = 0;
    h->err_index = 0;
    h->err_msg.clear();
    if (h->d_own) {
        spec_poll(h, true);
        h->spec_enabled = true;
        h->spec_batches = h->spec_fixed = h->spec_exact_frames = 0;
        HIP_TRY(h, hipMemsetAsync(h->d_spec_counters, 0, 4 * sizeof(uint32_t), h->stream));
    }
    if (h->d_lsummary) {
        if (h->lsummary_pending) { (void)hipEventSynchronize(h->lsummary_written); h->lsummary_pending = false; }
        h->decide_pause = 0;
        h->decide_submits = h->decide_paused_submits = 0;
        h->h_lsummary[0] = h->h_lsummary[1] = 0u;
        HIP_TRY(h, hipMemsetAsync(h->d_lsummary, 0, 2 * sizeof(uint32_t), h->stream));
    }
    return GORDER_OK;
}

int gorder_hip_comm_unique_id(uint8_t id[128]) {
    if (!id) return GORDER_ERR_INVALID_ARGUMENT;
    RcclApi *api = rccl_api(nullptr);
    if (!api) return GORDER_ERR_DEVICE;
    UniqueId u;
    if (api->get_unique_id(&u) != 0) return GORDER_ERR_DEVICE;
    memcpy(id, u.internal, 128);
    return GORDER_OK;
}

int gorder_hip_comm_create(gorder_hip_handle *h, const uint8_t id[128], int n_ranks, int rank, void **comm_out) {
    if (!h || !id || !comm_out || n_ranks < 1 || rank < 0 || rank >= n_ranks) return GORDER_ERR_INVALID_ARGUMENT;
    *comm_out = nullptr;
    std::string why;
    RcclApi *api = rccl_api(&why);
    if (!api) return fail(h, GORDER_ERR_DEVICE, why);
    HIP_TRY(h, hipSetDevice(h->device));
    UniqueId u;
    memcpy(u.internal, id, 128);
    const int rc = api->comm_init_rank(comm_out, n_ranks, u, rank);
    if (rc != 0) return fail(h, GORDER_ERR_DEVICE, rccl_error(api, "ncclCommInitRank", rc));
    return GORDER_OK;
}

void gorder_hip_comm_destroy(void *comm) {
    RcclApi *api = rccl_api(nullptr);
    if (api && comm) (void)api->comm_destroy(comm);
}

int gorder_hip_allreduce(gorder_hip_handle *h, void *nccl_comm) {
    if (!h || !nccl_comm) return GORDER_ERR_INVALID_ARGUMENT;
    std::string why;
    RcclApi *api = rccl_api(&why);
    if (!api) return fail(h, GORDER_ERR_DEVICE, why);
    HIP_TRY(h, hipSetDevice(h->device));
    int st = fold_replicas(h);
    if (st != GORDER_OK) return st;
    if ((st = fold_maps(h)) != GORDER_OK) return st;
    int rc = api->group_start();
    if (rc == 0) rc = api->all_reduce(h->d_acc, h->d_acc, h->acc_words, kNcclInt64, kNcclSum, nccl_comm, h->stream);
    if (rc == 0 && h->extra.maps) {
        const size_t nmap = 3 * (size_t)h->plan.n_acc * h->map_nx * h->map_ny;
        rc = api->all_reduce(h->d_map_sums, h->d_map_sums, nmap, kNcclInt64, kNcclSum, nccl_comm, h->stream);
        if (rc == 0) rc = api->all_reduce(h->d_map_cnts, h->d_map_cnts, nmap, kNcclInt64, kNcclSum, nccl_comm, h->stream);
    }
    const int rc_end = api->group_end();
    if (rc == 0) rc = rc_end;
    if (rc != 0) return fail(h, GORDER_ERR_DEVICE, rccl_error(api, "ncclAllReduce", rc));
    return GORDER_OK;
}

uint64_t gorder_hip_last_error_index(const gorder_hip_handle *h) { return h ? h->err_index : 0; }
uint64_t gorder_hip_last_error_frame(const gorder_hip_handle *h) { return h ? h->err_frame : 0; }
const char *gorder_hip_kernel_time_names(const gorder_hip_handle *h) { return h ? h->timed_kernels.c_str() : ""; }
const char *gorder_hip_last_error_message(const gorder_hip_handle *h) { return h ? h->err_msg.c_str() : ""; }

int gorder_hip_kernel_time(gorder_hip_handle *h, double *ms, uint64_t *launches, int reset) {
    if (!h) return GORDER_ERR_INVALID_ARGUMENT;
    HIP_TRY(h, hipSetDevice(h->device));
    h->timing_on = true;
    while (!h->timing_pending.empty()) {
        const int st = timing_drain_oldest(h);
        if (st != GORDER_OK) return st;
    }
    double total = 0.0;
    for (double v : h->timing_label_ms) total += v;
    if (ms) *ms = total;
    if (launches) *launches = h->timing_launches;
    if (reset) {
        h->timing_labels.clear(); h->timing_label_ms.clear(); h->timing_label_n.clear();
        h->timed_kernels.clear();
        h->timing_launches = 0;
        h->timing_open_label = -1;
    }
    return GORDER_OK;
}

int gorder_hip_kernel_time_group(gorder_hip_handle *h, uint32_t index, const char **name, double *ms, uint64_t *segments) {
    if (!h) return GORDER_ERR_INVALID_ARGUMENT;
    HIP_TRY(h, hipSetDevice(h->device));
    while (!h->timing_pending.empty()) {
        const int st = timing_drain_oldest(h);
        if (st != GORDER_OK) return st;
    }
    if (index >= h->timing_labels.size()) return GORDER_ERR_INVALID_ARGUMENT;
    if (name) *name = h->timing_labels[index].c_str();
    if (ms) *ms = h->timing_label_ms[index];
    if (segments) *segments = h->timing_label_n[index];
    return GORDER_OK;
}

size_t xtc_checkpoints(uint32_t n_frames, uint32_t n_stop) {
    return (size_t)n_frames * ((std::max(n_stop, 1u) + kXtcChunk - 1u) / kXtcChunk + 1u);
}
int xtc_decode_on(gorder_hip_handle *h, hipStream_t stream, const uint8_t *d_blob, uint64_t blob_bytes,
                  const gorder_xtc_frame_t *d_frames, uint32_t n_frames, uint32_t n_atoms_file, const int32_t *d_slot_of,
                  uint32_t n_stop, float *d_xyz, uint32_t n_atoms_out, uint32_t *d_stat = nullptr, uint32_t *d_short = nullptr,
                  uint32_t *d_err_key = nullptr, XtcCheckpoint *d_cp = nullptr) {
    if (!h || !d_blob || !d_frames || !d_xyz || blob_bytes < 64 || (reinterpret_cast<uintptr_t>(d_blob) & 63u) != 0 || n_atoms_file == 0 || n_atoms_out == 0 ||
        n_stop > n_atoms_file || (!d_slot_of && n_atoms_out < n_stop))
        return fail(h, GORDER_ERR_INVALID_ARGUMENT, "gorder_hip_xtc_decode: bad arguments");
    if (n_frames == 0) return GORDER_OK;
    HIP_TRY(h, hipSetDevice(h->device));
    const uint32_t n_chunks = (std::max(n_stop, 1u) + kXtcChunk - 1u) / kXtcChunk;
    if (!d_cp) {
        const int st = ensure(h, &h->d_xtc_cp, &h->xtc_cp_cap, xtc_checkpoints(n_frames, n_stop));
        if (st != GORDER_OK) return st;
        d_cp = h->d_xtc_cp;
    }
    hipLaunchKernelGGL(k_xtc_scan, dim3((n_frames + 3u) / 4u), dim3(256), 0, stream, d_blob, (unsigned long long)blob_bytes,
                       d_frames, n_frames, n_atoms_file, d_slot_of, n_stop, d_xyz, n_atoms_out,
                       d_err_key ? d_err_key : h->d_err, d_stat, d_short, d_cp, n_chunks);
    const unsigned long long items = (unsigned long long)n_frames * n_chunks;
    if (items + 63ull > 64ull * 0x7fffffffull) return fail(h, GORDER_ERR_INVALID_ARGUMENT, "gorder_hip_xtc_decode: batch too large");
    hipLaunchKernelGGL(k_xtc_chunks, dim3((uint32_t)((items + 63ull) / 64ull)), dim3(64), 0, stream, d_blob,
                       (unsigned long long)blob_bytes, d_frames, n_frames, n_atoms_file, d_slot_of, n_stop, d_xyz, n_atoms_out,
                       d_cp, n_chunks);
    HIP_TRY(h, hipGetLastError());
    return GORDER_OK;
}
int gorder_hip_xtc_decode(gorder_hip_handle *h, const uint8_t *d_blob, uint64_t blob_bytes,
                          const gorder_xtc_frame_t *d_frames, uint32_t n_frames, uint32_t n_atoms_file,
                          const int32_t *d_slot_of, uint32_t n_stop, float *d_xyz, uint32_t n_atoms_out) {
    if (!h) return GORDER_ERR_INVALID_ARGUMENT;
    return xtc_decode_on(h, h->stream, d_blob, blob_bytes, d_frames, n_frames, n_atoms_file, d_slot_of, n_stop, d_xyz,
                         n_atoms_out);
}

}

#include "trajectory_driver.h"
```

### gorder_amd/csrc/kernels_leaflets.h

```cpp
#pragma once

namespace {

struct LeafletArgs {
    const float *xyz;
    const float *box9;
    uint32_t n_atoms;
    const uint32_t *aframes;
    uint32_t row0;
    uint8_t *aflags;
    float *adist;
    uint32_t n_mol_total;
    const uint32_t *heads;
    const uint32_t *membrane;
    uint32_t n_membrane;
    const uint32_t *methyl_begin;
    const uint32_t *methyl_atoms;
    uint32_t dim;
    int flip, pbc;
    uint32_t *err;
    const uint8_t *skip;
    uint32_t n_assign;
};

// ... 442 lines not shown
        }
        __syncthreads();
        if (s_ok) {
            const float c = s_center;
            const bool last = f + 1 == a.n_frames;
            int bad = 0;
            for (uint32_t m = threadIdx.x; m < a.n_mol_total; m += blockDim.x) {
                float d = a.head_z[(size_t)f * a.n_mol_total + m] - c;
                if (a.pbc) d = gm_min_image(d, L, bad);
                a.aflags[(size_t)(1u + f) * a.n_mol_total + m] = (uint8_t)((d >= 0.0f ? 0 : 1) ^ (a.flip ? 1 : 0));
                if (last && a.adist) a.adist[m] = d;
            }
            if (bad) raise_box_range(a.err, f);
        }
        __syncthreads();
    }
}
struct SpecSample { uint32_t i, j, slot; };
template <bool ACOS_COS, bool TW>
__global__ __launch_bounds__(64) void k_spec_fixup(FrameArgs a, SpecArgs sa, const uint32_t *__restrict__ mol_begin,
                                                   const SpecSample *__restrict__ samples, unsigned long long *tw_sums,
                                                   unsigned long long *tw_cnts, uint64_t tw_row0) {
    const uint64_t n_pairs = (uint64_t)sa.n_frames * sa.n_mol_total;
    uint32_t moved = 0;
    for (uint64_t p0 = (uint64_t)blockIdx.x * 64u; p0 < n_pairs; p0 += (uint64_t)gridDim.x * 64u) {
        const uint64_t pi = p0 + threadIdx.x;
        bool differs = false;
        uint32_t exact_l = 0;
        if (pi < n_pairs) {
            exact_l = sa.aflags[(size_t)sa.n_mol_total + pi];
            differs = exact_l != sa.aflags[pi % sa.n_mol_total];
        }
        unsigned long long todo = __ballot(differs);
        moved += (uint32_t)__popcll(todo);
        while (todo) {
            const int l = __ffsll((long long)todo) - 1;
            todo &= todo - 1ull;
            const uint64_t pj = p0 + (uint64_t)l;
            const uint32_t f = (uint32_t)(pj / sa.n_mol_total), m = (uint32_t)(pj - (uint64_t)f * sa.n_mol_total);
            const uint32_t exact = (uint32_t)__shfl((int)exact_l, l, 64);
            const float *x = a.xyz + (size_t)f * a.n_atoms * 3u;
            for (uint32_t q = mol_begin[m] + threadIdx.x; q < mol_begin[m + 1]; q += 64u) {
                const SpecSample sm = samples[q];
                SampleAcc acc;
                int bad = 0;
                const float *p1 = x + 3u * (size_t)sm.i, *p2 = x + 3u * (size_t)sm.j;
                bond_sample<ACOS_COS>(a, f, p1[0], p1[1], p1[2], p2[0], p2[1], p2[2], m, acc, bad);
                unsigned long long *rep = a.rep;
                if (exact == 0u) {
                    atomicAdd(&rep[(size_t)a.n_acc + sm.slot], (unsigned long long)acc.s_tot);
                    atomicAdd(&rep[3u * (size_t)a.n_acc + sm.slot], 1ull);
                } else {
                    atomicAdd(&rep[(size_t)a.n_acc + sm.slot], (unsigned long long)(-acc.s_tot));
                    atomicAdd(&rep[3u * (size_t)a.n_acc + sm.slot], ~0ull);
                }
                if (TW) {
                    const size_t up = (size_t)(tw_row0 + f) * 3u * a.n_acc + (size_t)a.n_acc + sm.slot;
                    atomicAdd(&tw_sums[up], (unsigned long long)(exact == 0u ? acc.s_tot : -acc.s_tot));
                    atomicAdd(&tw_cnts[up], exact == 0u ? 1ull : ~0ull);
                }
            }
        }
    }
    if (threadIdx.x == 0u && moved) atomicAdd(&sa.counters[0], moved);
}
__global__ __launch_bounds__(256) void k_spec_finish(SpecArgs sa) {
    for (uint32_t m = threadIdx.x; m < sa.n_mol_total; m += blockDim.x)
        sa.aflags[m] = sa.aflags[(size_t)sa.n_frames * sa.n_mol_total + m];
    if (threadIdx.x == 0u) {
        sa.host_counters[0] = sa.counters[0];
        sa.host_counters[1] = sa.counters[1];
        sa.counters_next[0] = 0u;
        sa.counters_next[1] = 0u;
    }
}

__global__ __launch_bounds__(256) void k_leaflets_individual(LeafletArgs a) {
    const uint32_t m = blockIdx.x * blockDim.x + threadIdx.x;
    if (m >= a.n_mol_total) return;
    const uint32_t f = a.aframes[blockIdx.y];
    const float *x = a.xyz + (size_t)f * a.n_atoms * 3u;
    float L = 1.0f;
    if (a.pbc) L = a.box9[9 * (size_t)f + 4 * a.dim];
    int bad = 0;
    const float hp = x[3u * (size_t)a.heads[m] + a.dim];
    float total = 0.0f;
    for (uint32_t k = a.methyl_begin[m]; k < a.methyl_begin[m + 1]; k++) {
        const float mp = x[3u * (size_t)a.methyl_atoms[k] + a.dim];
        const float d = hp - mp;
        total += a.pbc ? gm_min_image(d, L, bad) : d;
    }
    a.aflags[(size_t)(a.row0 + blockIdx.y) * a.n_mol_total + m] =
        (uint8_t)((total >= 0.0f ? 0 : 1) ^ (a.flip ? 1 : 0));
    if (blockIdx.y + 1 == gridDim.y && a.adist) a.adist[m] = total;
    if (bad) raise_box_range(a.err, f);
}

constexpr uint32_t kLocalMaxCells1D = 128;
constexpr uint32_t kLocalSlabMax = 2048;
inline uint32_t local_slab_frames(size_t n_membrane) {
    const size_t per_frame = n_membrane * (2u * 12u + 4u) + (size_t)(2 * 4u + 16u + 16u) * kLocalMaxCells1D * (kLocalMaxCells1D + 1u) + 32u;
    const size_t n = ((size_t)4096 << 20) / per_frame;
    uint32_t cap = kLocalSlabMax;
    if (const char *ev = getenv("GORDER_HIP_LOCAL_SLAB")) cap = (uint32_t)std::max(4, atoi(ev));
    return (uint32_t)(n < 4 ? 4 : (n > cap ? cap : n));
}

struct LocalRowPre { float sc, ss; double sz; };
struct alignas(16) LocalEdge { uint32_t q; float zm, sq; uint32_t cs; };
constexpr uint32_t kEdgeSpanMax = 2000;
__device__ __forceinline__ uint32_t local_edge_trig(float sc, float ss) {
    return ((uint32_t)(int)__builtin_rintf(sc * 16.0f) & 0xffffu) | ((uint32_t)(int)__builtin_rintf(ss * 16.0f) << 16);
}
__device__ __forceinline__ void local_edge_trig_diff(uint32_t hi, uint32_t lo, float &dc, float &ds) {
    dc = (float)(int16_t)((hi & 0xffffu) - (lo & 0xffffu)) * 0.0625f;
    ds = (float)(int16_t)((hi >> 16) - (lo >> 16)) * 0.0625f;
}
struct LocalRec { float x, y, z; };

struct LocalArgs {
    const float *xyz;
    const float *box9;
    uint32_t n_atoms;
    const uint32_t *aframes;
    uint32_t frame0;
    uint32_t n_slab;
    uint32_t row0;
    uint8_t *aflags;
    float *adist;
    int write_dist_frame;
    uint32_t n_mol_total;
    const uint32_t *heads;
    const uint32_t *mol_slot0;
    const uint32_t *membrane;
    uint32_t n_membrane;
    uint4 *grid;
    uint32_t dim;
    int flip, pbc;
    float radius;
    float radius_thr;
    uint32_t *cell_of;
    float *trig;
    uint32_t *cell_count;
    uint32_t *cell_fill;
    int halo;
    int prune;
    uint32_t rows_groups;
    uint32_t rec_stride;
    LocalEdge *edge;
    LocalRowPre *rowpre;
    float4 *finfo;
    uint2 *todo;
    int sums;
    uint32_t *summary;
    uint32_t *summary_host;
    uint32_t *need;
    uint32_t *err;
};

constexpr uint32_t kLocalFine = 4;
constexpr uint32_t kLocalFineRows = 7;
__device__ __forceinline__ void local_axis(float L, float radius, uint32_t &nc, uint32_t &k, uint32_t k_max = kLocalFine,
                                           uint32_t nc_max = kLocalMaxCells1D) {
    nc = 1; k = 0;
    for (uint32_t kk = k_max; kk >= 1u; kk--) {
        const float fine = floorf(L / (radius / (float)kk) * 0.9999f);
        if (fine >= (float)(2u * kk + 1u) && fine <= (float)nc_max) { nc = (uint32_t)fine; k = kk; return; }
    }
}
__device__ __forceinline__ void local_grid(const LocalArgs &a, const float *box, uint32_t &nca, uint32_t &ncb,
                                           int &da, int &db, uint32_t &ka, uint32_t &kb) {
    da = (int)((a.dim + 1u) % 3u);
    db = (int)((a.dim + 2u) % 3u);
    nca = ncb = 1;
    ka = kb = 0;
    if (a.pbc) {
        const uint32_t k_max = a.halo ? kLocalFineRows : kLocalFine;
        local_axis(box[da], a.radius, nca, ka, k_max);
        local_axis(box[db], a.radius, ncb, kb, k_max, a.halo ? kLocalMaxCells1D - 2u * kLocalFineRows : kLocalMaxCells1D);
    }
}
__device__ __forceinline__ uint32_t local_row_stride(const LocalArgs &a, uint32_t ncb, uint32_t kb) {
    return a.halo ? ncb + 2u * kb : ncb;
}
__device__ __forceinline__ void local_grid(const LocalArgs &a, const float *box, uint32_t &nca, uint32_t &ncb,
                                           int &da, int &db) {
    uint32_t ka, kb;
    local_grid(a, box, nca, ncb, da, db, ka, kb);
}

__device__ __forceinline__ uint32_t local_float_key(float v) {
    const uint32_t b = __float_as_uint(v);
    return (b & 0x80000000u) ? ~b : (b | 0x80000000u);
}
__device__ __forceinline__ float local_key_float(uint32_t k) {
    return __uint_as_float((k & 0x80000000u) ? (k & 0x7fffffffu) : ~k);
}
__device__ __forceinline__ void local_finfo_init(const LocalArgs &a, uint32_t s) {
    if (a.finfo) reinterpret_cast<uint4 *>(a.finfo)[s] = make_uint4(0xffffffffu, 0u, 0u, 0u);
}
__device__ __forceinline__ void frame_box(const LocalArgs &a, uint32_t f, float *box) {
    box[0] = box[1] = box[2] = 1.0f;
    if (a.pbc) {
        const float *b = a.box9 + 9 * (size_t)f;
        box[0] = b[0]; box[1] = b[4]; box[2] = b[8];
    }
}

__device__ __forceinline__ uint32_t local_cell_of(const LocalArgs &a, uint32_t s, uint32_t f, uint32_t i,
                                                  const float *box, uint32_t nca, uint32_t ncb, uint32_t ncs, int da, int db) {
    const float *p = a.xyz + ((size_t)f * a.n_atoms + (a.membrane ? a.membrane[i] : i)) * 3u;
    int bad = 0;
    uint32_t ca = 0, cb = 0;
    if (a.pbc) {
        const float wa = gm_wrap(p[da], box[da], bad), wb = gm_wrap(p[db], box[db], bad);
        ca = (uint32_t)fminf(fmaxf(floorf(wa / box[da] * (float)nca), 0.0f), (float)(nca - 1u));
        cb = (uint32_t)fminf(fmaxf(floorf(wb / box[db] * (float)ncb), 0.0f), (float)(ncb - 1u));
    }
    const uint32_t c = ca * ncs + cb;
    a.cell_of[(size_t)s * a.n_membrane + i] = c;
    if (bad) raise_box_range(a.err, f);
    return c;
}

constexpr uint32_t kLocalLdsCells = 4096;

__global__ __launch_bounds__(256) void k_local_bin(LocalArgs a) {
    __shared__ uint32_t hist[kLocalLdsCells];
    const uint32_t i = blockIdx.x * blockDim.x + threadIdx.x;
    const uint32_t s = blockIdx.y;
    const uint32_t f = a.aframes ? a.aframes[s] : a.frame0 + s;
    float box[3];
    frame_box(a, f, box);
    uint32_t nca, ncb, ka, kb;
    int da, db;
    local_grid(a, box, nca, ncb, da, db, ka, kb);
    const uint32_t ncs = local_row_stride(a, ncb, kb), ncell = nca * ncs;
    uint32_t *count = a.cell_count + (size_t)s * (kLocalMaxCells1D * kLocalMaxCells1D + 1u);
    const bool lds = ncell <= kLocalLdsCells;
    if (lds) {
        for (uint32_t k = threadIdx.x; k < ncell; k += blockDim.x) hist[k] = 0;
        __syncthreads();
    }
    if (i < a.n_membrane) {
        const uint32_t c = local_cell_of(a, s, f, i, box, nca, ncb, ncs, da, db);
        if (lds) atomicAdd(&hist[c], 1u);
        else atomicAdd(&count[c], 1u);
        if (a.halo && c % ncs < 2u * kb) {
            if (lds) atomicAdd(&hist[c + ncb], 1u);
            else atomicAdd(&count[c + ncb], 1u);
        }
    }
    if (lds) {
        __syncthreads();
        for (uint32_t k = threadIdx.x; k < ncell; k += blockDim.x)
            if (hist[k]) atomicAdd(&count[k], hist[k]);
    }
}

__global__ __launch_bounds__(1024) void k_local_scan(LocalArgs a) {
    __shared__ uint32_t part[1024];
    const uint32_t s = blockIdx.x;
    uint32_t *cnt = a.cell_count + (size_t)s * (kLocalMaxCells1D * kLocalMaxCells1D + 1u);
    constexpr uint32_t N = kLocalMaxCells1D * kLocalMaxCells1D, PER = N / 1024u;
    uint32_t local[PER];
    uint32_t sum = 0;
    for (uint32_t k = 0; k < PER; k++) {
        local[k] = cnt[threadIdx.x * PER + k];
        sum += local[k];
    }
    part[threadIdx.x] = sum;
    __syncthreads();
    for (uint32_t off = 1; off < 1024; off <<= 1) {
        uint32_t v = threadIdx.x >= off ? part[threadIdx.x - off] : 0;
        __syncthreads();
        part[threadIdx.x] += v;
        __syncthreads();
    }
    uint32_t run = part[threadIdx.x] - sum;
    for (uint32_t k = 0; k < PER; k++) {
        cnt[threadIdx.x * PER + k] = run;
        run += local[k];
    }
    if (threadIdx.x == 1023) cnt[N] = run;
    if (threadIdx.x == 0 && a.grid) {
        float box[3];
        frame_box(a, a.aframes ? a.aframes[s] : a.frame0 + s, box);
        uint32_t nca, ncb, ka, kb;
        int da, db;
        local_grid(a, box, nca, ncb, da, db, ka, kb);
        a.grid[s] = make_uint4(nca, ncb, ka, kb);
        local_finfo_init(a, s);
    }
}

__global__ __launch_bounds__(256) void k_local_scatter(LocalArgs a) {
    __shared__ uint32_t hist[kLocalLdsCells];
    const uint32_t i = blockIdx.x * blockDim.x + threadIdx.x;
    const uint32_t s = blockIdx.y;
    const uint32_t f = a.aframes ? a.aframes[s] : a.frame0 + s;
    float box[3];
    frame_box(a, f, box);
    uint32_t nca, ncb, ka, kb;
    int da, db;
    local_grid(a, box, nca, ncb, da, db, ka, kb);
    const uint32_t ncs = local_row_stride(a, ncb, kb), ncell = nca * ncs;
// ... 764 lines not shown
        c_c = row_add<0x118>(c_c); c_s = row_add<0x118>(c_s);
        const float hm = hn_pos - z_mid, fn = (float)c_n, fr = (float)r_n, fi = (float)(c_n - r_n);
        const float T = c_z - fn * hm, A = r_z - fr * hm;
        const float B = __builtin_fmaxf((r_q - 2.0f * hm * r_z) + fr * hm * hm, 0.0f) * 1.02f + 1e-3f * fr;
        const float mid = T - 0.5f * A, rad = 0.5005f * __builtin_amdgcn_sqrtf(fr * B);
        const float slack = 0.1f + fn * (1e-3f + 1e-6f * fn * Ln);
        const float r_c = __builtin_amdgcn_sqrtf(c_c * c_c + c_s * c_s);
        const float est_c = (local_atan2_fast(-c_s, -c_c) + 3.1415927f) * (Ln * 0.15915494f);
        const float shift_c = gm_min_image(hn_pos - est_c, Ln, bad);
        const float xr = (fr + 1.0f) * __builtin_amdgcn_rcpf(r_c);
        const float emargin = 1e-4f * Ln + (xr + 0.5708f * xr * xr * xr) * (0.15916f * Ln);
        const bool same_image = fr + 1.0f < r_c && ulo_g + shift_c > -halfn + emargin && uhi_g + shift_c < halfn - emargin;
        const bool head_near = __builtin_fabsf(mid) + rad < (halfn - 1e-3f * Ln) * fi;
        const uint64_t wide = __ballot(!span_ok);
        const bool spans_ok = ((wide >> (16u * row)) & 0xffffull) == 0ull;
        const bool decided = !fail && !redo && spans_ok && c_n > r_n && same_image && head_near && (int)s != a.write_dist_frame &&
                             __builtin_fabsf(mid) > rad + slack;
        const uint64_t dm = __ballot(sub != 15u || decided || !head_ok);
        if (dm == ~0ull) {
            if (sub == 15u && head_ok)
                a.aflags[(size_t)(a.row0 + s) * a.n_mol_total + m] = (uint8_t)((mid > 0.0f ? 1 : 0) ^ (a.flip ? 1 : 0));
            if (bad) raise_box_range(a.err, f);
            return;
        }
    }
    if (try_prune && !fail && sub < n_rows && j_lo != j_hi) {
        const LocalRowPre p_lo = pre[row_e0 + j_lo], p_hi = pre[row_e0 + j_hi];
        sc += p_hi.sc - p_lo.sc;
        ss += p_hi.ss - p_lo.ss;
        inner_z = p_hi.sz - p_lo.sz;
    }
    {
        const uint32_t n_a = run_q1[0] - run_q0[0], n_b = run_q1[1] - run_q0[1];
        const uint32_t p_a = (n_a + 7u) >> 3, p_b = (n_b + 7u) >> 3, mine = p_a + p_b;
        uint32_t incl = mine;
        incl = row_add_u32<0x111>(incl); incl = row_add_u32<0x112>(incl); incl = row_add_u32<0x114>(incl); incl = row_add_u32<0x118>(incl);
        const uint32_t t0 = (uint32_t)__builtin_amdgcn_readlane((int)incl, 15), t1 = (uint32_t)__builtin_amdgcn_readlane((int)incl, 31);
        const uint32_t t2 = (uint32_t)__builtin_amdgcn_readlane((int)incl, 47), t3 = (uint32_t)__builtin_amdgcn_readlane((int)incl, 63);
        n_ring = row == 0u ? t0 : (row == 1u ? t1 : (row == 2u ? t2 : t3));
        constexpr uint32_t kRec = (uint32_t)sizeof(LocalRec);
        const uint32_t pos = incl - mine;
        const uint32_t a_from = run_q0[0] * kRec, a_to = run_q1[0] * kRec, b_from = run_q0[1] * kRec, b_to = run_q1[1] * kRec;
        for (uint32_t k = 0; k < mine; k++) {
            const bool second = k >= p_a;
            const uint32_t from = (second ? b_from - p_a * (8u * kRec) : a_from) + k * (8u * kRec), to = second ? b_to : a_to;
            if (pos + k < kRowRing) ring[pos + k] = make_uint2(from, min(to, from + 8u * kRec));
        }
    }
    redo |= n_ring > kRowRing;
    uint32_t n_max = max(max((uint32_t)__builtin_amdgcn_readlane((int)n_ring, 0), (uint32_t)__builtin_amdgcn_readlane((int)n_ring, 16)),
                         max((uint32_t)__builtin_amdgcn_readlane((int)n_ring, 32), (uint32_t)__builtin_amdgcn_readlane((int)n_ring, 48)));
    n_max = min(n_max, kRowRing);
    const uint32_t n_mine = min(n_ring, kRowRing), half = sub >> 3, lane_off = (sub & 7u) * (uint32_t)sizeof(LocalRec);
    const uint32_t n_end = (n_max + 2u * kRowFlight - 1u) / (2u * kRowFlight) * (2u * kRowFlight);
    for (uint32_t e = n_mine + sub; e < n_end; e += 16u) ring[e] = make_uint2(0u, 0u);
    __builtin_amdgcn_wave_barrier();
    const __amdgpu_buffer_rsrc_t rec_rsrc = __builtin_amdgcn_make_buffer_rsrc(const_cast<LocalRec *>(rec), 0, a.rec_stride * (uint32_t)sizeof(LocalRec), 0x00020000);
    typedef uint32_t u3 __attribute__((ext_vector_type(3)));
    typedef float f3 __attribute__((ext_vector_type(3)));
    float t_min = 0.0f;
    for (uint32_t t = 0; !fail && t < n_max; t += 2u * kRowFlight) {
        f3 r[kRowFlight];
        uint2 run[kRowFlight];
        bool v[kRowFlight];
#pragma unroll
        for (uint32_t u = 0; u < kRowFlight; u++) run[u] = ring[t + 2u * u + half];
#pragma unroll
        for (uint32_t u = 0; u < kRowFlight; u++) {
            const uint32_t q = run[u].x + lane_off;
            v[u] = q < run[u].y;
            r[u] = __builtin_bit_cast(f3, (u3)__builtin_amdgcn_raw_buffer_load_b96(rec_rsrc, (int)q, 0, 0));
        }
#pragma unroll
        for (uint32_t u = 0; u < kRowFlight; u++) {
            const float ea = __builtin_fabsf(r[u].x - ha_pos), eb = __builtin_fabsf(r[u].y - hb_pos);
            const float ta = La - ea, tb = Lb - eb;
            const float ma = __builtin_fminf(ea, ta), mb = __builtin_fminf(eb, tb);
            const bool in = v[u] & (ma * ma + mb * mb < thr);
            t_min = __builtin_fminf(t_min, __builtin_fminf(ta, tb));
            cnt += in ? 1u : 0u;
            su += in ? r[u].z : 0.0f;
        }
    }
    redo |= t_min < 0.0f;
    double tu = (double)su + inner_z;
    tu = row_add_f64<0x111>(tu); tu = row_add_f64<0x112>(tu); tu = row_add_f64<0x114>(tu); tu = row_add_f64<0x118>(tu);
    sc = row_add<0x111>(sc); ss = row_add<0x111>(ss); cnt = row_add_u32<0x111>(cnt); n_inner = row_add_u32<0x111>(n_inner);
    sc = row_add<0x112>(sc); ss = row_add<0x112>(ss); cnt = row_add_u32<0x112>(cnt); n_inner = row_add_u32<0x112>(n_inner);
    sc = row_add<0x114>(sc); ss = row_add<0x114>(ss); cnt = row_add_u32<0x114>(cnt); n_inner = row_add_u32<0x114>(n_inner);
    sc = row_add<0x118>(sc); ss = row_add<0x118>(ss); cnt = row_add_u32<0x118>(cnt); n_inner = row_add_u32<0x118>(n_inner);
    const uint64_t redo_mask = __ballot(redo);
    const bool row_redo = ((redo_mask >> (16u * row)) & 0xffffull) != 0ull;
    bool general = fail || row_redo;
    if (sub == 15u && head_ok && !general) {
        if (cnt == 0u) {
            raise_error(a.err, GORDER_ERR_INVALID_LOCAL_MEMBRANE_CENTER, f, kStageTypes, a.mol_slot0 ? a.mol_slot0[m] : 0u, 0, m);
        } else {
            const float r_inner = __builtin_amdgcn_sqrtf(sc * sc + ss * ss), e_ring = (float)(cnt - n_inner) + 1.0f;
            const float est = (local_atan2_fast(-ss, -sc) + 3.1415927f) * (Ln * 0.15915494f);
            const float shift = gm_min_image(hn_pos - est, Ln, bad);
            const float margin = 1e-4f * Ln + e_ring * __builtin_amdgcn_rcpf(r_inner) * (0.2501f * Ln);
            if (e_ring < r_inner && ulo_g + shift > -halfn + margin && uhi_g + shift < halfn - margin) {
                const double dc = (double)cnt;
                double rc = __builtin_amdgcn_rcp(dc);
                rc = __builtin_fma(__builtin_fma(-dc, rc, 1.0), rc, rc);
                rc = __builtin_fma(__builtin_fma(-dc, rc, 1.0), rc, rc);
                const float center = gm_wrap((float)(tu * rc), Ln, bad);
                if (center != center) {
                    raise_error(a.err, GORDER_ERR_INVALID_LOCAL_MEMBRANE_CENTER, f, kStageTypes, a.mol_slot0 ? a.mol_slot0[m] : 0u, 0, m);
                } else {
                    const float d = gm_min_image(hn_pos - center, Ln, bad);
                    a.aflags[(size_t)(a.row0 + s) * a.n_mol_total + m] = (uint8_t)((d >= 0.0f ? 0 : 1) ^ (a.flip ? 1 : 0));
                    if ((int)s == a.write_dist_frame && a.adist) a.adist[m] = d;
                }
            } else {
                general = true;
            }
        }
    }
    if (bad) raise_box_range(a.err, f);
    if (general && head_ok && sub == 15u) {
        const uint32_t at = atomicAdd(&a.todo[0].x, 1u);
        a.todo[1u + at] = make_uint2(s, m);
    }
}
constexpr uint32_t kRowsSlots = 1;
__global__ __launch_bounds__(256) void k_local_flags_rows(LocalArgs a) {
    __shared__ LocalRingLists l_ring[16];
    const uint32_t n_groups = a.rows_groups, linear = blockIdx.x;
    const uint32_t xcd = linear & 7u, k = linear >> 3;
    const uint32_t s = (k / n_groups) * 8u + xcd, bx = k - (k / n_groups) * n_groups;
    if (s < a.n_slab) local_rows_group(a, s, bx, l_ring);
}
__global__ __launch_bounds__(256) void k_local_flags_rows_open(LocalArgs a) {
    __shared__ LocalRingLists l_ring[16];
    const uint32_t n_groups = a.rows_groups, linear = blockIdx.x;
    const uint32_t xcd = linear & 7u, k = linear >> 3;
    if (a.need[a.n_slab] == 0u) return;
    const uint32_t slot = k / n_groups, bx = k - slot * n_groups, lane = threadIdx.x & 63u;
    uint32_t seen = 0;
    for (uint32_t base = xcd; base < a.n_slab; base += 8u * 64u) {
        const uint32_t sl = base + 8u * lane;
        uint64_t open = __ballot(sl < a.n_slab && a.need[sl] != 0u);
        while (open != 0ull) {
            const uint32_t bit = (uint32_t)__builtin_ctzll(open);
            open &= open - 1ull;
            if (seen++ % kRowsSlots == slot) local_rows_group(a, (uint32_t)__builtin_amdgcn_readfirstlane((int)(base + 8u * bit)), bx, l_ring);
        }
    }
}

constexpr uint32_t kSumsCells = 9000;
constexpr uint32_t kSumsLds = kSumsCells * 2u * (uint32_t)sizeof(unsigned long long);
struct LocalWrapped { float a, b; int bad; };
__device__ __attribute__((noinline)) LocalWrapped local_wrap_far(float xa, float xb, float La, float Lb) {
    LocalWrapped w;
    w.bad = 0;
    w.a = gm_wrap(xa, La, w.bad);
    w.b = gm_wrap(xb, Lb, w.bad);
    return w;
}
__device__ __forceinline__ uint32_t wave_scan_u32(uint32_t v, uint32_t lane) {
    v = row_add_u32<0x111>(v); v = row_add_u32<0x112>(v); v = row_add_u32<0x114>(v); v = row_add_u32<0x118>(v);
    const uint32_t t0 = (uint32_t)__builtin_amdgcn_readlane((int)v, 15), t1 = (uint32_t)__builtin_amdgcn_readlane((int)v, 31),
                   t2 = (uint32_t)__builtin_amdgcn_readlane((int)v, 47);
    const uint32_t r = lane >> 4;
    return v + (r > 0u ? t0 : 0u) + (r > 1u ? t1 : 0u) + (r > 2u ? t2 : 0u);
}
__device__ __forceinline__ double wave_scan_f64(double v, uint32_t lane) {
    v = row_add_f64<0x111>(v); v = row_add_f64<0x112>(v); v = row_add_f64<0x114>(v); v = row_add_f64<0x118>(v);
    const double t0 = lane_value(v, 15), t1 = lane_value(v, 31), t2 = lane_value(v, 47);
    const uint32_t r = lane >> 4;
    return v + (r > 0u ? t0 : 0.0) + (r > 1u ? t1 : 0.0) + (r > 2u ? t2 : 0.0);
}
__global__ __launch_bounds__(1024) void k_local_sums(LocalArgs a) {
    extern __shared__ unsigned long long l_sums[];
    __shared__ float l_zlo[16], l_zhi[16];
    __shared__ uint32_t l_flag[16];
    const uint32_t s = blockIdx.x, tid = threadIdx.x, lane = tid & 63u, wave = tid >> 6;
    const uint32_t f = a.aframes ? a.aframes[s] : a.frame0 + s;
    float box[3];
    frame_box(a, f, box);
    uint32_t nca, ncb, ka, kb;
    int da, db;
    local_grid(a, box, nca, ncb, da, db, ka, kb);
    const uint32_t ncs = local_row_stride(a, ncb, kb), n_base = nca * ncb;
    const int dn = (int)a.dim;
    if (tid == 0u) a.grid[s] = make_uint4(nca, ncb, ka, kb);
    if (!(a.pbc && ka >= 1u && kb >= 1u && n_base <= kSumsCells)) {
        if (tid == 0u) { local_finfo_init(a, s); a.need[s] = 1u; a.need[a.n_slab] = 1u; }
        return;
    }
    unsigned long long *l_a = l_sums, *l_b = l_sums + n_base;
    for (uint32_t k = tid; k < 2u * n_base; k += 1024u) l_sums[k] = 0ull;
    __syncthreads();
    const float *x = a.xyz + (size_t)f * a.n_atoms * 3u;
    const float La = box[da], Lb = box[db], Ln = box[dn];
    const float inv_a = (float)nca / La, inv_b = (float)ncb / Lb, inv_Ln = 1.0f / Ln, z_mid = 0.5f * Ln;
    int bad = 0;
    float zlo = 3.0e38f, zhi = -3.0e38f;
    uint32_t flag = 0;
    constexpr uint32_t U = 8;
    for (uint32_t i0 = tid; i0 < a.n_membrane; i0 += U * 1024u) {
        uint32_t at[U];
        float pa[U], pb[U], pn[U];
#pragma unroll
        for (uint32_t u = 0; u < U; u++) { const uint32_t i = min(i0 + u * 1024u, a.n_membrane - 1u); at[u] = a.membrane ? a.membrane[i] : i; }
#pragma unroll
        for (uint32_t u = 0; u < U; u++) {
            pa[u] = x[3u * (size_t)at[u] + da]; pb[u] = x[3u * (size_t)at[u] + db]; pn[u] = x[3u * (size_t)at[u] + dn];
        }
#pragma unroll
        for (uint32_t u = 0; u < U; u++) {
            if (i0 + u * 1024u >= a.n_membrane) continue;
            float wa = pa[u] > La ? pa[u] - La : pa[u], wb = pb[u] > Lb ? pb[u] - Lb : pb[u];
            wa = wa < 0.0f ? wa + La : wa;
            wb = wb < 0.0f ? wb + Lb : wb;
            if (__builtin_expect(!(wa >= 0.0f && wa <= La && wb >= 0.0f && wb <= Lb), 0)) {
                const LocalWrapped w = local_wrap_far(pa[u], pb[u], La, Lb);
                wa = w.a; wb = w.b; bad |= w.bad;
            }
            const uint32_t ca = (uint32_t)fminf(fmaxf(floorf(wa * inv_a), 0.0f), (float)(nca - 1u));
            const uint32_t cb = (uint32_t)fminf(fmaxf(floorf(wb * inv_b), 0.0f), (float)(ncb - 1u));
            const float z = pn[u], zm = z - z_mid;
            float sn, cs;
            local_trig(z, inv_Ln, &sn, &cs);
            const bool finite = ((pa[u] - pa[u]) + (pb[u] - pb[u])) + (z - z) == 0.0f;
            const bool room = zm > -8.0f && zm < 8.0f;
            flag |= (finite ? 0u : 1u) | (room ? 0u : 2u);
            zlo = fminf(zlo, z);
            zhi = fmaxf(zhi, z);
            if (finite && room) {
                const unsigned long long wa64 = ((unsigned long long)(uint32_t)__builtin_rintf((zm + 8.0f) * 32768.0f) << 32) |
                                                (unsigned long long)(uint32_t)__builtin_rintf(zm * zm * 8192.0f);
                const unsigned long long wb64 = (1ull << 42) | ((unsigned long long)(uint32_t)__builtin_rintf((cs + 1.0f) * 256.0f) << 21) |
                                                (unsigned long long)(uint32_t)__builtin_rintf((sn + 1.0f) * 256.0f);
                atomicAdd(&l_a[ca * ncb + cb], wa64);
                atomicAdd(&l_b[ca * ncb + cb], wb64);
            }
        }
    }
    if (bad) raise_box_range(a.err, f);
    __syncthreads();
    LocalEdge *out = a.edge + (size_t)s * (kLocalMaxCells1D * (kLocalMaxCells1D + 1u));
    for (uint32_t ra = wave; ra < nca; ra += 16u) {
        uint32_t c_n = 0, c_c = 0, c_s = 0;
        double c_z = 0.0, c_q = 0.0;
        for (uint32_t j0 = 0; j0 <= ncs; j0 += 64u) {
            const uint32_t j = j0 + lane, jb = j < ncb ? j : j - ncb;
            unsigned long long va = 0ull, vb = 0ull;
            if (j < ncs) { va = l_a[ra * ncb + jb]; vb = l_b[ra * ncb + jb]; }
            const uint32_t n = (uint32_t)(vb >> 42), ci = (uint32_t)(vb >> 21) & 0x1fffffu, si = (uint32_t)vb & 0x1fffffu;
            const double zi = (double)(uint32_t)(va >> 32), qi = (double)(uint32_t)va;
            flag |= n > 4095u ? 2u : 0u;
            const uint32_t i_n = wave_scan_u32(n, lane), i_c = wave_scan_u32(ci, lane), i_s = wave_scan_u32(si, lane);
            const double i_z = wave_scan_f64(zi, lane), i_q = wave_scan_f64(qi, lane);
            if (j <= ncs) {
                const uint32_t e_n = c_n + (i_n - n);
                const double e_z = c_z + (i_z - zi), e_q = c_q + (i_q - qi);
                const float e_c = (float)(c_c + (i_c - ci)) * (1.0f / 256.0f) - (float)e_n;
                const float e_s = (float)(c_s + (i_s - si)) * (1.0f / 256.0f) - (float)e_n;
                LocalEdge e;
                e.q = e_n;
                e.zm = (float)(e_z * (1.0 / 32768.0) - 8.0 * (double)e_n);
                e.sq = (float)(e_q * (1.0 / 8192.0));
                e.cs = local_edge_trig(e_c, e_s);
                out[(size_t)ra * (ncs + 1u) + j] = e;
            }
            c_n += (uint32_t)__builtin_amdgcn_readlane((int)i_n, 63);
            c_c += (uint32_t)__builtin_amdgcn_readlane((int)i_c, 63);
            c_s += (uint32_t)__builtin_amdgcn_readlane((int)i_s, 63);
            c_z += lane_value(i_z, 63);
            c_q += lane_value(i_q, 63);
        }
    }
    for (int off = 32; off >= 1; off >>= 1) {
        zlo = fminf(zlo, __shfl_xor(zlo, off, 64));
        zhi = fmaxf(zhi, __shfl_xor(zhi, off, 64));
        flag |= (uint32_t)__shfl_xor((int)flag, off, 64);
    }
    if (lane == 0u) { l_zlo[wave] = zlo; l_zhi[wave] = zhi; l_flag[wave] = flag; }
    __syncthreads();
    if (tid == 0u) {
        for (uint32_t w = 1; w < 16u; w++) { zlo = fminf(zlo, l_zlo[w]); zhi = fmaxf(zhi, l_zhi[w]); flag |= l_flag[w]; }
        reinterpret_cast<uint4 *>(a.finfo)[s] = zlo <= zhi ? make_uint4(local_float_key(zlo), local_float_key(zhi), flag & 1u, 2u)
                                                            : make_uint4(0xffffffffu, 0u, flag & 1u, 2u);
        if (flag) { a.need[s] = 1u; a.need[a.n_slab] = 1u; }
    }
}

constexpr uint32_t kDecideEntries = 10000;
constexpr uint32_t kDecideLds = kDecideEntries * (uint32_t)sizeof(LocalEdge);
struct DecideFrame {
    uint32_t nca, ncb, ka, kb, ncs, n_rows;
    int da, db, dn;
    float La, Lb, Ln, z_min, z_max;
};
template <typename EdgePtr>
__device__ __forceinline__ bool local_decide_head(const LocalArgs &a, const DecideFrame &F, uint32_t f, uint32_t m, EdgePtr edge,
                                                  bool &centre_above, int &bad) {
    const uint32_t nca = F.nca, ncb = F.ncb, ka = F.ka, kb = F.kb, ncs = F.ncs, n_rows = F.n_rows;
    const float La = F.La, Lb = F.Lb, Ln = F.Ln;
    const float halfn = Ln / 2.0f, z_mid = 0.5f * Ln;
    const float thr = a.radius_thr;
    const float *hp = a.xyz + ((size_t)f * a.n_atoms + a.heads[m]) * 3u;
    const float ha_pos = hp[F.da], hb_pos = hp[F.db], hn_pos = hp[F.dn];
    const float wa = ha_pos < 0.0f ? ha_pos + La : (ha_pos > La ? ha_pos - La : ha_pos);
    const float wb = hb_pos < 0.0f ? hb_pos + Lb : (hb_pos > Lb ? hb_pos - Lb : hb_pos);
    const float ca = La * __builtin_amdgcn_rcpf((float)nca), cb = Lb * __builtin_amdgcn_rcpf((float)ncb);
    const uint32_t ha = (uint32_t)fminf(fmaxf(floorf(wa * __builtin_amdgcn_rcpf(ca)), 0.0f), (float)(nca - 1u));
    const uint32_t hb = (uint32_t)fminf(fmaxf(floorf(wb * __builtin_amdgcn_rcpf(cb)), 0.0f), (float)(ncb - 1u));
    const float fa = wa - (float)ha * ca, fb = wb - (float)hb * cb;
    uint32_t a0 = ha + nca - ka, b0 = hb + ncb - kb;
    a0 -= a0 >= nca ? nca : 0u;
    b0 -= b0 >= ncb ? ncb : 0u;
    const float ulo_g = F.z_min - hn_pos, uhi_g = F.z_max - hn_pos;
    const bool redo = !(fa >= -1e-4f * ca && fa <= ca * 1.0001f && fb >= -1e-4f * cb && fb <= cb * 1.0001f) ||
                      !(wa >= 0.0f && wa <= La && wb >= 0.0f && wb <= Lb);
    const float r_in = thr * (1.0f - 4e-4f), r_out = thr * (1.0f + 4e-4f);
    const float inv_cb = __builtin_amdgcn_rcpf(cb), t0 = fb * inv_cb + (float)kb, two_kb = (float)(2u * kb);
    uint32_t c_n = 0, r_n = 0;
    float c_z = 0.0f, r_z = 0.0f, r_q = 0.0f, c_c = 0.0f, c_s = 0.0f;
    bool spans_ok = true;
    for (uint32_t sub0 = 0; sub0 < n_rows; sub0 += 4u) {
        LocalEdge e_a[4], e_d[4], e_lo[4], e_hi[4];
#pragma unroll
        for (uint32_t u = 0; u < 4u; u++) {
            const uint32_t sub = sub0 + u;
            const float a_lo = ((float)sub - (float)ka) * ca - fa, a_hi = a_lo + ca;
            const float a_far = fmaxf(fabsf(a_lo), fabsf(a_hi));
            const float a_near = (a_lo <= 0.0f && a_hi >= 0.0f) ? 0.0f : fminf(fabsf(a_lo), fabsf(a_hi));
            const float w_out2 = r_out - a_near * a_near, w_in2 = r_in - a_far * a_far;
            const bool touch = sub < n_rows && w_out2 > 0.0f;
            const float w_out = __builtin_amdgcn_sqrtf(fmaxf(w_out2, 0.0f)) * inv_cb;
            const float jo_lo_f = floorf(t0 - w_out - 1e-3f), jo_hi_f = floorf(t0 + w_out + 1e-3f);
            const uint32_t jo_lo = (uint32_t)fminf(fmaxf(jo_lo_f, 0.0f), two_kb);
            const uint32_t jo_hi = (uint32_t)fminf(fmaxf(jo_hi_f, 0.0f), two_kb);
            const float w_in = __builtin_amdgcn_sqrtf(fmaxf(w_in2, 0.0f)) * inv_cb;
            const float lo_f = ceilf(t0 - w_in + 1e-3f), hi_f = floorf(t0 + w_in - 1e-3f) - 1.0f;
            const bool inner = w_in2 > 0.0f && hi_f >= lo_f;
            const uint32_t ji_lo = (uint32_t)fmaxf(lo_f, (float)jo_lo), ji_hi = (uint32_t)fmaxf(fminf(hi_f, (float)jo_hi), 0.0f);
            const bool has_inner = inner && ji_lo <= ji_hi;
            const uint32_t j_d = jo_hi + 1u;
            const uint32_t j_lo = has_inner ? ji_lo : j_d, j_hi = has_inner ? ji_hi + 1u : j_d;
            uint32_t ra = a0 + (sub < n_rows ? sub : 0u);
            ra -= ra >= nca ? nca : 0u;
            EdgePtr row_edge = edge + (ra * (ncs + 1u) + b0);
            e_a[u] = row_edge[touch ? jo_lo : 0u];
            e_d[u] = row_edge[touch ? j_d : 0u];
            e_lo[u] = row_edge[touch ? j_lo : 0u];
            e_hi[u] = row_edge[touch ? j_hi : 0u];
        }
#pragma unroll
        for (uint32_t u = 0; u < 4u; u++) {
            const uint32_t n_c = e_d[u].q - e_a[u].q;
            const float z_c = e_d[u].zm - e_a[u].zm;
            c_n += n_c;
            c_z += z_c;
            r_n += n_c - (e_hi[u].q - e_lo[u].q);
            r_z += z_c - (e_hi[u].zm - e_lo[u].zm);
            r_q += (e_d[u].sq - e_a[u].sq) - (e_hi[u].sq - e_lo[u].sq);
            float dc, ds;
            local_edge_trig_diff(e_d[u].cs, e_a[u].cs, dc, ds);
            c_c += dc;
            c_s += ds;
            spans_ok &= n_c < kEdgeSpanMax;
        }
    }
    const float hm = hn_pos - z_mid, fn = (float)c_n, fr = (float)r_n, fi = (float)(c_n - r_n);
    const float T = c_z - fn * hm, A = r_z - fr * hm;
    const float B = __builtin_fmaxf((r_q - 2.0f * hm * r_z) + fr * hm * hm, 0.0f) * 1.02f + 1e-3f * fr;
    const float mid = T - 0.5f * A, rad = 0.5005f * __builtin_amdgcn_sqrtf(fr * B);
    const float slack = 0.1f + fn * (1.05e-3f + 1e-6f * fn * Ln);
    const float r_c = __builtin_amdgcn_sqrtf(c_c * c_c + c_s * c_s);
    const float est_c = (local_atan2_fast(-c_s, -c_c) + 3.1415927f) * (Ln * 0.15915494f);
    const float shift_c = gm_min_image(hn_pos - est_c, Ln, bad);
    const float e_c = fr + 1.0f + 0.004f * fn;
    const float xr = e_c * __builtin_amdgcn_rcpf(r_c);
    const float emargin = 1e-4f * Ln + (xr + 0.5708f * xr * xr * xr) * (0.15916f * Ln);
    const bool same_image = e_c < r_c && ulo_g + shift_c > -halfn + emargin && uhi_g + shift_c < halfn - emargin;
    const bool head_near = __builtin_fabsf(mid) + rad < (halfn - 1e-3f * Ln) * fi;
    centre_above = mid > 0.0f;
    return !redo && spans_ok && c_n > r_n && same_image && head_near && a.prune != 2 &&
           __builtin_fabsf(mid) > rad + slack;
}
template <typename EdgePtr>
__device__ __forceinline__ void local_decide_frame(const LocalArgs &a, const DecideFrame &F, uint32_t s, uint32_t f, EdgePtr edge) {
    int bad = 0;
    uint32_t n_open = 0;
    for (uint32_t m0 = threadIdx.x & ~63u; m0 < a.n_mol_total; m0 += 1024u) {
        const uint32_t m_raw = m0 + (threadIdx.x & 63u);
        const bool head_ok = m_raw < a.n_mol_total;
        const uint32_t m = head_ok ? m_raw : a.n_mol_total - 1u;
        bool centre_above;
        const bool decided = local_decide_head(a, F, f, m, edge, centre_above, bad);
        if (decided && head_ok)
            a.aflags[(size_t)(a.row0 + s) * a.n_mol_total + m] = (uint8_t)((centre_above ? 1 : 0) ^ (a.flip ? 1 : 0));
        n_open += (uint32_t)__popcll(__ballot(!decided && head_ok));
    }
    if (n_open != 0u && (threadIdx.x & 63u) == 0u) { atomicAdd(&a.need[s], n_open); a.need[a.n_slab] = 1u; }
    if (bad) raise_box_range(a.err, f);
}
__global__ __launch_bounds__(1024) void k_local_decide(LocalArgs a) {
    extern __shared__ LocalEdge l_edge[];
    const uint32_t s = blockIdx.x;
    const uint32_t f = a.aframes ? a.aframes[s] : a.frame0 + s;
    float box[3];
    frame_box(a, f, box);
    const uint4 g = a.grid[s];
    const uint4 fk = reinterpret_cast<const uint4 *>(a.finfo)[s];
    DecideFrame F;
    F.nca = g.x; F.ncb = g.y; F.ka = g.z; F.kb = g.w; F.ncs = g.y + 2u * g.w; F.n_rows = 2u * g.z + 1u;
    F.da = (int)((a.dim + 1u) % 3u); F.db = (int)((a.dim + 2u) % 3u); F.dn = (int)a.dim;
    F.La = box[F.da]; F.Lb = box[F.db]; F.Ln = box[F.dn];
    F.z_min = local_key_float(fk.x); F.z_max = local_key_float(fk.y);
    const bool fail = !(F.ka >= 1u && F.kb >= 1u && F.n_rows <= 16u && fk.z == 0u && fk.x <= fk.y);
    if (a.sums && s == 0u && threadIdx.x == 0u) a.todo[0] = make_uint2(0u, 0u);
    if (fail || !(F.z_max - F.z_min < 0.75f * F.Ln) || (int)s == a.write_dist_frame || (a.sums && a.need[s] != 0u)) {
        if (threadIdx.x == 0u) { atomicAdd(&a.need[s], 1u); a.need[a.n_slab] = 1u; }
        return;
    }
    const LocalEdge *edge = a.edge + (size_t)s * (kLocalMaxCells1D * (kLocalMaxCells1D + 1u));
    const uint32_t n_entries = F.nca * (F.ncs + 1u);
    if (n_entries <= kDecideEntries) {
        const uint4 *src = reinterpret_cast<const uint4 *>(edge);
        uint4 *dst = reinterpret_cast<uint4 *>(l_edge);
        for (uint32_t i = threadIdx.x; i < n_entries; i += 1024u) dst[i] = src[i];
        __syncthreads();
        local_decide_frame<const LocalEdge *>(a, F, s, f, l_edge);
    } else {
        local_decide_frame<const LocalEdge *>(a, F, s, f, edge);
    }
}

__global__ __launch_bounds__(256) void k_local_flags_todo(LocalArgs a) {
    if (a.need && a.summary && blockIdx.x == 0u && threadIdx.x < 64u) {
        uint32_t c = 0;
        for (uint32_t s = threadIdx.x; s < a.n_slab; s += 64u) c += a.need[s] != 0u ? 1u : 0u;
        c = wave_total_u32(c);
        if (threadIdx.x == 0u) {
            const uint32_t open = atomicAdd(&a.summary[0], c) + c, seen = atomicAdd(&a.summary[1], a.n_slab) + a.n_slab;
            if (a.summary_host) {
                a.summary_host[0] = open;
                a.summary_host[1] = seen;
                a.summary[0] = a.summary[1] = 0u;
            }
        }
    }
    const uint32_t n = a.todo[0].x;
    for (uint32_t i = blockIdx.x * 4u + (threadIdx.x >> 6); i < n; i += gridDim.x * 4u) {
        const uint2 e = a.todo[1u + i];
        local_flags_head(a, (uint32_t)__builtin_amdgcn_readfirstlane((int)e.x), (uint32_t)__builtin_amdgcn_readfirstlane((int)e.y));
    }
}

constexpr int kSphKeep = 16;
constexpr int kSphMaxIter = 50;
constexpr float kSphTolerance = 1e-4f;

struct SphArgs {
    const float *xyz;
    const float *box9;
    uint32_t n_atoms;
    const uint32_t *aframes;
    uint32_t row0;
    uint32_t n_assign;
    uint8_t *aflags;
    float *adist;
    float *stats;
    uint32_t n_mol_total;
    const uint32_t *heads;
    const uint32_t *group;
    uint32_t n_group;
    int flip, pbc;
    float *spill;
    uint32_t n_spill;
    uint32_t *err;
};

struct SphParams { float w, mean_a, var_a, mean_b, var_b; };

template <int N>
__device__ __forceinline__ void block_sum_n(double (&v)[N], double *scratch) {
    const uint32_t wave = threadIdx.x >> 6, n_waves = (blockDim.x + 63u) >> 6;
#pragma unroll
    for (int q = 0; q < N; q++) {
        v[q] = wave_sum(v[q]);
        if ((threadIdx.x & 63u) == 0) scratch[16 * q + wave] = v[q];
    }
    __syncthreads();
#pragma unroll
    for (int q = 0; q < N; q++) {
        double r = 0.0;
        for (uint32_t w = 0; w < n_waves; w++) r += scratch[16 * q + w];
        v[q] = r;
    }
    __syncthreads();
}

__device__ __forceinline__ float sph_distance(const float *p, const float (&c)[3], const float (&box)[3], int pbc, int &bad) {
    float v[3];
#pragma unroll
    for (int d = 0; d < 3; d++) {
        const float dx = p[d] - c[d];
        v[d] = pbc ? gm_min_image(dx, box[d], bad) : dx;
    }
    return __builtin_sqrtf((v[0] * v[0] + v[1] * v[1]) + v[2] * v[2]);
}

__device__ __forceinline__ float sph_log_gaussian(float x, float mean, float log_var, float var) {
    const float diff = x - mean;
    return -0.5f * ((1.8378770664093453f + log_var) + diff * diff / var);
}
struct SphEStep { float log_wa, log_wb, log_va, log_vb; };
__device__ __forceinline__ SphEStep sph_estep_setup(const SphParams &p) {
    return {logf(p.w), logf(1.0f - p.w), logf(p.var_a), logf(p.var_b)};
}
__device__ __forceinline__ float sph_responsibility(float x, const SphParams &p, const SphEStep &e, float &log_px) {
    const float ja = e.log_wa + sph_log_gaussian(x, p.mean_a, e.log_va, p.var_a);
    const float jb = e.log_wb + sph_log_gaussian(x, p.mean_b, e.log_vb, p.var_b);
    const float m = fmaxf(ja, jb);
    log_px = m + logf(expf(ja - m) + expf(jb - m));
    return expf(ja - log_px);
}

template <uint32_t THREADS>
__global__ __launch_bounds__(THREADS) void k_leaflets_spherical(SphArgs a) {
    __shared__ double scratch[6 * 16];
    __shared__ uint32_t hist[2][256];
    __shared__ uint32_t s_pref[2], s_rank[2];
    const uint32_t bi = blockIdx.x, tid = threadIdx.x, n = a.n_group;
    const uint32_t f = a.aframes[bi];
    const float *x = a.xyz + (size_t)f * a.n_atoms * 3u;
    float *spill = a.spill + (size_t)bi * a.n_spill;
    uint8_t *row = a.aflags + (size_t)(a.row0 + bi) * a.n_mol_total;
    const bool last = bi + 1u == a.n_assign;
    float box[3] = {1.0f, 1.0f, 1.0f};
    if (a.pbc) { const float *b = a.box9 + 9 * (size_t)f; box[0] = b[0]; box[1] = b[4]; box[2] = b[8]; }
    int bad = 0;

    float est[3] = {0.0f, 0.0f, 0.0f};
    if (a.pbc) {
        double cs[6] = {0, 0, 0, 0, 0, 0};
        float inv[3];
#pragma unroll
        for (int d = 0; d < 3; d++) inv[d] = 1.0f / box[d];
        for (uint32_t i = tid; i < n; i += THREADS) {
            const float *p = x + 3u * (size_t)a.group[i];
#pragma unroll
            for (int d = 0; d < 3; d++) {
                float sn, c;
                fast_sincos_rev(gm_wrap(p[d], box[d], bad) * inv[d], &sn, &c);
                cs[d] += (double)c;
                cs[3 + d] += (double)sn;
            }
        }
        block_sum_n<6>(cs, scratch);
#pragma unroll
        for (int d = 0; d < 3; d++) est[d] = (atan2f(-(float)cs[3 + d], -(float)cs[d]) + 3.1415927f) / (6.2831855f / box[d]);
    }
    float centre[3];
    {
        double acc[3] = {0, 0, 0};
        for (uint32_t i = tid; i < n; i += THREADS) {
            const float *p = x + 3u * (size_t)a.group[i];
#pragma unroll
            for (int d = 0; d < 3; d++) acc[d] += (double)(a.pbc ? gm_nearest_image(p[d], est[d], box[d], bad) : p[d]);
        }
// ... 160 lines not shown
```

### include/gorder_hip.h

```cpp
#ifndef GORDER_HIP_H
#define GORDER_HIP_H

#include <stddef.h>
#include <stdint.h>

#include "gorder_xtc.h"

#ifdef __cplusplus
extern "C" {
#endif

typedef enum {
    GORDER_OK = 0,
    GORDER_ERR_UNDEFINED_BOX = 1,
    GORDER_ERR_NOT_ORTHOGONAL_BOX = 2,
    GORDER_ERR_ZERO_BOX = 3,
    GORDER_ERR_UNDEFINED_POSITION = 4,
    GORDER_ERR_INVALID_GLOBAL_MEMBRANE_CENTER = 5,
    GORDER_ERR_INVALID_LOCAL_MEMBRANE_CENTER = 6,
    GORDER_ERR_DYNAMIC_NORMAL = 7,
    GORDER_ERR_INVALID_ARGUMENT = 100,
    GORDER_ERR_DEVICE = 101,
    GORDER_ERR_NO_DEVICE = 102,
    GORDER_ERR_BOX_RANGE = 103,
// ... 64 lines not shown
typedef enum { GORDER_GEOM_NONE = 0, GORDER_GEOM_CUBOID = 1, GORDER_GEOM_CYLINDER = 2, GORDER_GEOM_SPHERE = 3 } gorder_geom_kind_t;
typedef enum { GORDER_GEOMREF_POINT = 0, GORDER_GEOMREF_BOX_CENTER = 1, GORDER_GEOMREF_GROUP = 2 } gorder_geom_ref_t;
typedef struct {
    uint32_t kind;
    uint32_t invert;
    uint32_t reference;
    float point[3];
    uint32_t n_group;
    const uint32_t *group;
    float xdim[2], ydim[2], zdim[2];
    float radius;
    float span[2];
    uint32_t orientation;
    float structure_box[3];
} gorder_geometry_t;

typedef enum {
    GORDER_FLAG_TRIG_ACOS_COS = 1u,
    GORDER_FLAG_UA_FAST_NORMALISE = 2u
} gorder_flags_t;

typedef struct {
    uint32_t n_atoms;
    uint32_t n_molecule_types;
    const gorder_moltype_t *molecule_types;
    int32_t handle_pbc;
    float normal[3];
    gorder_leaflets_t leaflets;
    gorder_ordermap_t ordermap;
    int32_t timewise;
    int32_t device;
    uint32_t flags;
    gorder_geometry_t geometry;
    gorder_dynamic_normal_t dynamic_normal;
} gorder_tables_t;


typedef struct gorder_hip_handle gorder_hip_handle;

int gorder_hip_create(const gorder_tables_t *tables, gorder_hip_handle **out);
void gorder_hip_destroy(gorder_hip_handle *h);

uint32_t gorder_hip_n_accumulators(const gorder_hip_handle *h);
uint32_t gorder_hip_ordermap_dims(const gorder_hip_handle *h, uint32_t *nx, uint32_t *ny);

int gorder_hip_set_stream(gorder_hip_handle *h, void *hip_stream);

int gorder_hip_submit_device(gorder_hip_handle *h, const float *d_xyz, const float *d_box,
                             const uint64_t *frame_index, uint32_t n_frames);

int gorder_hip_submit_host(gorder_hip_handle *h, const float *xyz, const float *box,
                           const uint64_t *frame_index, uint32_t n_frames);

typedef struct {
    const char *const *paths;
    uint32_t n_paths;
    const uint32_t *group;
    uint32_t n_group;
    float begin_ps, end_ps;
    uint32_t step;
    uint32_t n_threads;
    uint32_t batch_frames;
    uint64_t first_frame_index;
    uint32_t device_decode;
    uint32_t shard_index;
    uint32_t shard_count;
    uint32_t reserved;
} gorder_trajectory_t;

typedef struct {
    uint64_t n_frames;
    uint64_t n_batches;
    uint64_t bytes_h2d;
    double seconds_total;
    double seconds_decode;
    double seconds_reader_stalled;
    double seconds_gpu_starved;
    uint32_t batch_frames, decoder_threads;
    uint32_t device_decode;
    uint32_t frames_decoded_by_host;
    uint64_t shard_first, shard_frames_total;
    double seconds_setup;
} gorder_trajectory_stats_t;

int gorder_hip_run_trajectory(gorder_hip_handle *h, const gorder_trajectory_t *trajectory,
                              gorder_trajectory_stats_t *stats );
void gorder_hip_release_staging(gorder_hip_handle *h);

int gorder_hip_xtc_decode(gorder_hip_handle *h, const uint8_t *d_blob, uint64_t blob_bytes,
                          const gorder_xtc_frame_t *d_frames, uint32_t n_frames, uint32_t n_atoms_file,
                          const int32_t *d_slot_of, uint32_t n_stop, float *d_xyz, uint32_t n_atoms_out);

int gorder_hip_prime_leaflets(gorder_hip_handle *h, const float *d_xyz, const float *d_box,
                              uint64_t frame_index);

int gorder_hip_set_manual_leaflets(gorder_hip_handle *h, const uint8_t *flags, uint64_t frame_index);

int gorder_hip_synchronize(gorder_hip_handle *h);

int gorder_hip_finish(gorder_hip_handle *h, int64_t *sums, uint64_t *counts, int64_t *map_sums,
                      uint64_t *map_counts, uint64_t *n_frames_analyzed);

int gorder_hip_timewise(gorder_hip_handle *h, int64_t *tw_sums, uint64_t *tw_counts,
                        uint64_t capacity_frames);

int gorder_hip_leaflets(gorder_hip_handle *h, uint8_t *flags, uint64_t *assignment_frame);
int gorder_hip_leaflet_distances(gorder_hip_handle *h, float *distances);
int gorder_hip_spherical_stats(gorder_hip_handle *h, float out[12]);

int gorder_hip_set_normals(gorder_hip_handle *h, const float *normals, uint32_t n_frames);

int gorder_hip_normals(gorder_hip_handle *h, float *normals, uint32_t *n_points);

int gorder_hip_accumulators_device(gorder_hip_handle *h, void **d_ptr, uint64_t *n_u64);

int gorder_hip_comm_unique_id(uint8_t id[128]);
int gorder_hip_comm_create(gorder_hip_handle *h, const uint8_t id[128], int n_ranks, int rank, void **comm_out);
void gorder_hip_comm_destroy(void *comm);
int gorder_hip_allreduce(gorder_hip_handle *h, void *nccl_comm);

int gorder_hip_reset(gorder_hip_handle *h);

int gorder_hip_export_maps(gorder_hip_handle *h, void *d_sums, void *d_counts, uint64_t n_u64);

int gorder_hip_bind_accumulators(gorder_hip_handle *h, void *d_ptr, uint64_t n_u64);

uint64_t gorder_hip_last_error_index(const gorder_hip_handle *h);
uint64_t gorder_hip_last_error_frame(const gorder_hip_handle *h);
const char *gorder_hip_last_error_message(const gorder_hip_handle *h);
const char *gorder_hip_strerror(int status);

int gorder_hip_kernel_time(gorder_hip_handle *h, double *ms, uint64_t *launches, int reset);
int gorder_hip_kernel_time_group(gorder_hip_handle *h, uint32_t index, const char **name, double *ms, uint64_t *segments);
const char *gorder_hip_kernel_time_names(const gorder_hip_handle *h);

typedef struct {
    uint32_t n_tiles;
    uint32_t block_threads;
    uint32_t max_window_atoms;
    uint32_t n_direct_items;
    uint32_t frames_per_stage;
    uint32_t lds_bytes;
    uint32_t map_staged;
    uint32_t map_lds_bytes;
    uint32_t leaflets_one_read;
} gorder_hip_plan_t;
int gorder_hip_plan(const gorder_hip_handle *h, gorder_hip_plan_t *plan);
int gorder_hip_plan_tables(const gorder_tables_t *tables, gorder_hip_plan_t *plan, int *selfcheck);

int gorder_hip_speculation_stats(gorder_hip_handle *h, uint64_t out[4]);

int gorder_hip_local_decide_stats(gorder_hip_handle *h, uint64_t out[4]);

int gorder_hip_selftest_arithmetic(int device, uint64_t n, uint64_t seed, uint64_t mismatches[2]);
int gorder_hip_selftest_trig(int device, int fn, uint32_t first_bits, uint32_t stride, uint32_t n, float *out);

#ifdef __cplusplus
}
#endif
#endif
```

Baseline: 20.94 million.

## Add flat-membrane local sums path skipping trig accumulation, specialize on normal axis

Result: no change. 21.04 million, median of 6 (+0.5%).

```diff
diff --git a/gorder_amd/abi.py b/gorder_amd/abi.py
--- a/gorder_amd/abi.py
+++ b/gorder_amd/abi.py
@@ -295,7 +295,7 @@
     "gorder_hip_plan_tables", "gorder_hip_selftest_arithmetic", "gorder_hip_selftest_trig", "gorder_hip_run_trajectory",
     "gorder_hip_comm_unique_id", "gorder_hip_comm_create", "gorder_hip_comm_destroy", "gorder_hip_allreduce",
     "gorder_hip_reset", "gorder_hip_xtc_decode", "gorder_hip_release_staging", "gorder_hip_speculation_stats", "gorder_hip_local_decide_stats",
-    "gorder_hip_spherical_stats",
+    "gorder_hip_spherical_stats", "gorder_hip_local_sums_stats",
 ]
 
 _lib = None
@@ -362,6 +362,7 @@
     lib.gorder_hip_plan.argtypes = [vp, C.POINTER(CPlan)]
     lib.gorder_hip_speculation_stats.argtypes = [vp, C.POINTER(C.c_uint64)]
     lib.gorder_hip_local_decide_stats.argtypes = [vp, C.POINTER(C.c_uint64)]
+    lib.gorder_hip_local_sums_stats.argtypes = [vp, C.POINTER(C.c_uint64)]
     lib.gorder_hip_spherical_stats.argtypes = [vp, C.POINTER(C.c_float)]
     lib.gorder_hip_plan_tables.argtypes = [C.POINTER(CTables), C.POINTER(CPlan), C.POINTER(i32)]
     lib.gorder_hip_selftest_arithmetic.argtypes = [i32, C.c_uint64, C.c_uint64, C.POINTER(C.c_uint64)]
@@ -672,6 +673,11 @@
         self._check(self.lib.gorder_hip_local_decide_stats(self._h, out))
         return {"submits": int(out[0]), "paused": int(out[1]), "open_frames": int(out[2]), "frames": int(out[3])}
 
+    def local_sums_stats(self) -> dict:
+        out = (C.c_uint64 * 4)()
+        self._check(self.lib.gorder_hip_local_sums_stats(self._h, out))
+        return {"flat_frames": int(out[0]), "redone_frames": int(out[1]), "workgroups_per_cu": int(out[2]), "levers": int(out[3])}
+
     def spherical_stats(self) -> dict:
         out = (C.c_float * 12)()
         self._check(self.lib.gorder_hip_spherical_stats(self._h, out))
diff --git a/gorder_amd/csrc/gorder_hip.hip b/gorder_amd/csrc/gorder_hip.hip
--- a/gorder_amd/csrc/gorder_hip.hip
+++ b/gorder_amd/csrc/gorder_hip.hip
@@ -62,6 +62,9 @@
     float4 *d_lfinfo = nullptr;
     static constexpr uint32_t kDecidePause = 16;
     uint32_t *d_lsummary = nullptr, *h_lsummary = nullptr;
+    uint32_t local_sums_levers = 3;
+    uint32_t *d_lsums_stats = nullptr;
+    int local_sums_per_cu = 0;
     hipEvent_t lsummary_written = nullptr;
     bool lsummary_pending = false;
     uint32_t decide_pause = 0;
@@ -1141,8 +1144,19 @@
                 HIP_TRY(h, hipEventCreateWithFlags(&h->lsummary_written, hipEventDisableTiming));
                 HIP_TRY(h, hipFuncSetAttribute(reinterpret_cast<const void *>(k_local_decide), hipFuncAttributeMaxDynamicSharedMemorySize,
                                                (int)kDecideLds));
-                HIP_TRY(h, hipFuncSetAttribute(reinterpret_cast<const void *>(k_local_sums), hipFuncAttributeMaxDynamicSharedMemorySize,
-                                               (int)kSumsLds));
+                if (const char *lv = std::getenv("GORDER_HIP_LOCAL_SUMS_LEVERS")) h->local_sums_levers = (uint32_t)std::strtoul(lv, nullptr, 0) & 3u;
+                for (const void *fn : {reinterpret_cast<const void *>(k_local_sums<-1, false>), reinterpret_cast<const void *>(k_local_sums<0, false>),
+                                       reinterpret_cast<const void *>(k_local_sums<1, false>), reinterpret_cast<const void *>(k_local_sums<2, false>)})
+                    HIP_TRY(h, hipFuncSetAttribute(fn, hipFuncAttributeMaxDynamicSharedMemorySize, (int)kSumsLds));
+                for (const void *fn : {reinterpret_cast<const void *>(k_local_sums<-1, true>), reinterpret_cast<const void *>(k_local_sums<0, true>),
+                                       reinterpret_cast<const void *>(k_local_sums<1, true>), reinterpret_cast<const void *>(k_local_sums<2, true>)})
+                    HIP_TRY(h, hipFuncSetAttribute(fn, hipFuncAttributeMaxDynamicSharedMemorySize, (int)kFlatLds));
+                if (hipOccupancyMaxActiveBlocksPerMultiprocessor(&h->local_sums_per_cu, k_local_sums<2, true>, 1024, kFlatLds) != hipSuccess) {
+                    (void)hipGetLastError();
+                    h->local_sums_per_cu = 0;
+                }
+                HIP_TRY(h, hipMalloc((void **)&h->d_lsums_stats, 2 * sizeof(uint32_t)));
+                HIP_TRY(h, hipMemset(h->d_lsums_stats, 0, 2 * sizeof(uint32_t)));
                 HIP_TRY(h, hipMalloc((void **)&h->d_ltodo, (1 + sl * (size_t)(p.n_mol_total ? p.n_mol_total : 1)) * sizeof(uint2)));
             }
         }
@@ -1172,6 +1186,7 @@
     (void)hipFree(h->d_spec_counters); (void)hipFree(h->d_spec_mol_begin); (void)hipFree(h->d_spec_samples);
     if (h->h_spec_counters) (void)hipHostFree(h->h_spec_counters);
     for (hipEvent_t ev : h->spec_counters_copied) if (ev) (void)hipEventDestroy(ev); (void)hipFree(h->d_lfinfo); (void)hipFree(h->d_ltodo); (void)hipFree(h->d_lneed);
+    (void)hipFree(h->d_lsums_stats);
     (void)hipFree(h->d_lsummary); if (h->h_lsummary) (void)hipHostFree(h->h_lsummary); if (h->lsummary_written) (void)hipEventDestroy(h->lsummary_written);
     (void)hipFree(h->d_dyn_cloud); (void)hipFree(h->d_dyn_heads); (void)hipFree(h->d_dyn_cell_of); (void)hipFree(h->d_dyn_count);
     (void)hipFree(h->d_dyn_rec); (void)hipFree(h->d_dyn_normals); (void)hipFree(h->d_dyn_cov);
@@ -1227,6 +1242,16 @@
     return GORDER_OK;
 }
 
+int gorder_hip_local_sums_stats(gorder_hip_handle *h, uint64_t out[4]) {
+    if (!h || !out) return GORDER_ERR_INVALID_ARGUMENT;
+    HIP_TRY(h, hipSetDevice(h->device));
+    HIP_TRY(h, hipStreamSynchronize(h->stream));
+    uint32_t c[2] = {0u, 0u};
+    if (h->d_lsums_stats) HIP_TRY(h, hipMemcpy(c, h->d_lsums_stats, sizeof(c), hipMemcpyDeviceToHost));
+    out[0] = c[0]; out[1] = c[1]; out[2] = (uint64_t)h->local_sums_per_cu; out[3] = h->local_sums_levers;
+    return GORDER_OK;
+}
+
 int gorder_hip_plan(const gorder_hip_handle *h, gorder_hip_plan_t *plan) {
     if (!h || !plan) return GORDER_ERR_INVALID_ARGUMENT;
     plan->n_tiles = (uint32_t)h->plan.tiles.size();
@@ -1254,6 +1279,24 @@
             h->spec_enabled = false;
         h->spec_ring_frames[i] = 0;
     }
+}
+
+static void launch_local_sums(gorder_hip_handle *h, LocalArgs lo, uint32_t ns, uint32_t n_membrane) {
+    const bool flat = (h->local_sums_levers & 2u) != 0u && n_membrane <= kFlatMaxAtoms;
+    const int dn = (h->local_sums_levers & 1u) != 0u ? (int)lo.dim : -1;
+#define LOCAL_SUMS_LAUNCH(DN)                                                                                         \
+    do {                                                                                                              \
+        if (flat) {                                                                                                   \
+            hipLaunchKernelGGL((k_local_sums<DN, true>), dim3(ns), dim3(1024), kFlatLds, h->stream, lo);              \
+            lo.sums = 2;                                                                                              \
+        }                                                                                                             \
+        hipLaunchKernelGGL((k_local_sums<DN, false>), dim3(ns), dim3(1024), kSumsLds, h->stream, lo);                 \
+    } while (0)
+    if (dn == 0) LOCAL_SUMS_LAUNCH(0);
+    else if (dn == 1) LOCAL_SUMS_LAUNCH(1);
+    else if (dn == 2) LOCAL_SUMS_LAUNCH(2);
+    else LOCAL_SUMS_LAUNCH(-1);
+#undef LOCAL_SUMS_LAUNCH
 }
 
 static int run_leaflets(gorder_hip_handle *h, const float *d_xyz, const float *d_box,
@@ -1342,6 +1385,7 @@
         lo.edge = h->d_ledge;
         lo.finfo = h->d_lfinfo;
         lo.todo = h->d_ltodo;
+        lo.sums_stats = h->d_lsums_stats;
         bool decide = lo.halo && lo.prune && lo.n_mol_total && !env_flag("GORDER_HIP_LOCAL_NO_DECIDE");
         if (decide) {
             if (h->lsummary_pending) {
@@ -1372,7 +1416,7 @@
             if (lo.sums) {
                 HIP_TRY(h, hipMemsetAsync(h->d_lneed, 0, (ns + 1) * sizeof(uint32_t), h->stream));
                 TIMING_MARK(h, "k_local_sums");
-                hipLaunchKernelGGL(k_local_sums, dim3(ns), dim3(1024), kSumsLds, h->stream, lo);
+                launch_local_sums(h, lo, ns, lf.n_membrane);
                 TIMING_MARK(h, "k_local_decide");
                 hipLaunchKernelGGL(k_local_decide, dim3(ns), dim3(1024), kDecideLds, h->stream, lo);
             }
@@ -1867,6 +1911,7 @@
         h->h_lsummary[0] = h->h_lsummary[1] = 0u;
         HIP_TRY(h, hipMemsetAsync(h->d_lsummary, 0, 2 * sizeof(uint32_t), h->stream));
     }
+    if (h->d_lsums_stats) HIP_TRY(h, hipMemsetAsync(h->d_lsums_stats, 0, 2 * sizeof(uint32_t), h->stream));
     return GORDER_OK;
 }
 
diff --git a/gorder_amd/csrc/kernels_leaflets.h b/gorder_amd/csrc/kernels_leaflets.h
--- a/gorder_amd/csrc/kernels_leaflets.h
+++ b/gorder_amd/csrc/kernels_leaflets.h
@@ -618,6 +618,7 @@
     float4 *finfo;
     uint2 *todo;
     int sums;
+    uint32_t *sums_stats;
     uint32_t *summary;
     uint32_t *summary_host;
     uint32_t *need;
@@ -1688,6 +1689,10 @@
 
 constexpr uint32_t kSumsCells = 9000;
 constexpr uint32_t kSumsLds = kSumsCells * 2u * (uint32_t)sizeof(unsigned long long);
+constexpr uint32_t kFlatCells = 8000;
+constexpr uint32_t kFlatLds = kFlatCells * (uint32_t)sizeof(unsigned long long) + kFlatCells / 2u * (uint32_t)sizeof(uint32_t);
+constexpr uint32_t kFlatMaxAtoms = 65535;
+constexpr float kFlatExtent = 0.53f;
 struct LocalWrapped { float a, b; int bad; };
 __device__ __attribute__((noinline)) LocalWrapped local_wrap_far(float xa, float xb, float La, float Lb) {
     LocalWrapped w;
@@ -1709,11 +1714,13 @@
     const uint32_t r = lane >> 4;
     return v + (r > 0u ? t0 : 0.0) + (r > 1u ? t1 : 0.0) + (r > 2u ? t2 : 0.0);
 }
-__global__ __launch_bounds__(1024) void k_local_sums(LocalArgs a) {
+template <int DN, bool FLAT>
+__global__ __launch_bounds__(1024, FLAT ? 8 : 1) void k_local_sums(LocalArgs a) {
     extern __shared__ unsigned long long l_sums[];
     __shared__ float l_zlo[16], l_zhi[16];
     __shared__ uint32_t l_flag[16];
     const uint32_t s = blockIdx.x, tid = threadIdx.x, lane = tid & 63u, wave = tid >> 6;
+    if (!FLAT && a.sums == 2 && reinterpret_cast<const uint4 *>(a.finfo)[s].w != 10u) return;
     const uint32_t f = a.aframes ? a.aframes[s] : a.frame0 + s;
     float box[3];
     frame_box(a, f, box);
@@ -1721,14 +1728,24 @@
     int da, db;
     local_grid(a, box, nca, ncb, da, db, ka, kb);
     const uint32_t ncs = local_row_stride(a, ncb, kb), n_base = nca * ncb;
-    const int dn = (int)a.dim;
+    const int dn = DN >= 0 ? DN : (int)a.dim;
     if (tid == 0u) a.grid[s] = make_uint4(nca, ncb, ka, kb);
     if (!(a.pbc && ka >= 1u && kb >= 1u && n_base <= kSumsCells)) {
         if (tid == 0u) { local_finfo_init(a, s); a.need[s] = 1u; a.need[a.n_slab] = 1u; }
         return;
     }
+    if (FLAT && n_base > kFlatCells) {
+        if (tid == 0u) { reinterpret_cast<uint4 *>(a.finfo)[s] = make_uint4(0xffffffffu, 0u, 0u, 10u); atomicAdd(&a.sums_stats[1], 1u); }
+        return;
+    }
     unsigned long long *l_a = l_sums, *l_b = l_sums + n_base;
-    for (uint32_t k = tid; k < 2u * n_base; k += 1024u) l_sums[k] = 0ull;
+    uint32_t *l_n = reinterpret_cast<uint32_t *>(l_sums + n_base);
+    if (FLAT) {
+        for (uint32_t k = tid; k < n_base; k += 1024u) l_a[k] = 0ull;
+        for (uint32_t k = tid; k < (n_base + 1u) / 2u; k += 1024u) l_n[k] = 0u;
+    } else {
+        for (uint32_t k = tid; k < 2u * n_base; k += 1024u) l_sums[k] = 0ull;
+    }
     __syncthreads();
     const float *x = a.xyz + (size_t)f * a.n_atoms * 3u;
     const float La = box[da], Lb = box[db], Ln = box[dn];
@@ -1736,7 +1753,7 @@
     int bad = 0;
     float zlo = 3.0e38f, zhi = -3.0e38f;
     uint32_t flag = 0;
-    constexpr uint32_t U = 8;
+    constexpr uint32_t U = FLAT ? 4 : 8;
     for (uint32_t i0 = tid; i0 < a.n_membrane; i0 += U * 1024u) {
         uint32_t at[U];
         float pa[U], pb[U], pn[U];
@@ -1744,7 +1761,13 @@
         for (uint32_t u = 0; u < U; u++) { const uint32_t i = min(i0 + u * 1024u, a.n_membrane - 1u); at[u] = a.membrane ? a.membrane[i] : i; }
 #pragma unroll
         for (uint32_t u = 0; u < U; u++) {
-            pa[u] = x[3u * (size_t)at[u] + da]; pb[u] = x[3u * (size_t)at[u] + db]; pn[u] = x[3u * (size_t)at[u] + dn];
+            if (DN >= 0) {
+                const float *p = x + 3u * (size_t)at[u];
+                const float v[3] = {p[0], p[1], p[2]};
+                pa[u] = v[(DN + 1) % 3]; pb[u] = v[(DN + 2) % 3]; pn[u] = v[DN % 3];
+            } else {
+                pa[u] = x[3u * (size_t)at[u] + da]; pb[u] = x[3u * (size_t)at[u] + db]; pn[u] = x[3u * (size_t)at[u] + dn];
+            }
         }
 #pragma unroll
         for (uint32_t u = 0; u < U; u++) {
@@ -1759,25 +1782,40 @@
             const uint32_t ca = (uint32_t)fminf(fmaxf(floorf(wa * inv_a), 0.0f), (float)(nca - 1u));
             const uint32_t cb = (uint32_t)fminf(fmaxf(floorf(wb * inv_b), 0.0f), (float)(ncb - 1u));
             const float z = pn[u], zm = z - z_mid;
-            float sn, cs;
-            local_trig(z, inv_Ln, &sn, &cs);
             const bool finite = ((pa[u] - pa[u]) + (pb[u] - pb[u])) + (z - z) == 0.0f;
             const bool room = zm > -8.0f && zm < 8.0f;
             flag |= (finite ? 0u : 1u) | (room ? 0u : 2u);
             zlo = fminf(zlo, z);
             zhi = fmaxf(zhi, z);
             if (finite && room) {
+                const uint32_t cell = ca * ncb + cb;
                 const unsigned long long wa64 = ((unsigned long long)(uint32_t)__builtin_rintf((zm + 8.0f) * 32768.0f) << 32) |
                                                 (unsigned long long)(uint32_t)__builtin_rintf(zm * zm * 8192.0f);
-                const unsigned long long wb64 = (1ull << 42) | ((unsigned long long)(uint32_t)__builtin_rintf((cs + 1.0f) * 256.0f) << 21) |
-                                                (unsigned long long)(uint32_t)__builtin_rintf((sn + 1.0f) * 256.0f);
-                atomicAdd(&l_a[ca * ncb + cb], wa64);
-                atomicAdd(&l_b[ca * ncb + cb], wb64);
+                atomicAdd(&l_a[cell], wa64);
+                if (FLAT) {
+                    atomicAdd(&l_n[cell >> 1], 1u << (16u * (cell & 1u)));
+                } else {
+                    float sn, cs;
+                    local_trig(z, inv_Ln, &sn, &cs);
+                    const unsigned long long wb64 = (1ull << 42) | ((unsigned long long)(uint32_t)__builtin_rintf((cs + 1.0f) * 256.0f) << 21) |
+                                                    (unsigned long long)(uint32_t)__builtin_rintf((sn + 1.0f) * 256.0f);
+                    atomicAdd(&l_b[cell], wb64);
+                }
             }
         }
     }
     if (bad) raise_box_range(a.err, f);
+    for (int off = 32; off >= 1; off >>= 1) {
+        zlo = fminf(zlo, __shfl_xor(zlo, off, 64));
+        zhi = fmaxf(zhi, __shfl_xor(zhi, off, 64));
+    }
+    if (lane == 0u) { l_zlo[wave] = zlo; l_zhi[wave] = zhi; }
     __syncthreads();
+    for (uint32_t w = 0; w < 16u; w++) { zlo = fminf(zlo, l_zlo[w]); zhi = fmaxf(zhi, l_zhi[w]); }
+    if (FLAT && !(zhi - zlo < kFlatExtent * Ln)) {
+        if (tid == 0u) { reinterpret_cast<uint4 *>(a.finfo)[s] = make_uint4(0xffffffffu, 0u, 0u, 10u); atomicAdd(&a.sums_stats[1], 1u); }
+        return;
+    }
     LocalEdge *out = a.edge + (size_t)s * (kLocalMaxCells1D * (kLocalMaxCells1D + 1u));
     for (uint32_t ra = wave; ra < nca; ra += 16u) {
         uint32_t c_n = 0, c_c = 0, c_s = 0;
@@ -1785,43 +1823,54 @@
         for (uint32_t j0 = 0; j0 <= ncs; j0 += 64u) {
             const uint32_t j = j0 + lane, jb = j < ncb ? j : j - ncb;
             unsigned long long va = 0ull, vb = 0ull;
-            if (j < ncs) { va = l_a[ra * ncb + jb]; vb = l_b[ra * ncb + jb]; }
-            const uint32_t n = (uint32_t)(vb >> 42), ci = (uint32_t)(vb >> 21) & 0x1fffffu, si = (uint32_t)vb & 0x1fffffu;
+            uint32_t n = 0, ci = 0, si = 0;
+            if (j < ncs) {
+                const uint32_t cell = ra * ncb + jb;
+                va = l_a[cell];
+                if (FLAT) n = (l_n[cell >> 1] >> (16u * (cell & 1u))) & 0xffffu;
+                else vb = l_b[cell];
+            }
+            if (!FLAT) { n = (uint32_t)(vb >> 42); ci = (uint32_t)(vb >> 21) & 0x1fffffu; si = (uint32_t)vb & 0x1fffffu; }
             const double zi = (double)(uint32_t)(va >> 32), qi = (double)(uint32_t)va;
             flag |= n > 4095u ? 2u : 0u;
-            const uint32_t i_n = wave_scan_u32(n, lane), i_c = wave_scan_u32(ci, lane), i_s = wave_scan_u32(si, lane);
+            const uint32_t i_n = wave_scan_u32(n, lane);
+            uint32_t i_c = 0, i_s = 0;
+            if (!FLAT) { i_c = wave_scan_u32(ci, lane); i_s = wave_scan_u32(si, lane); }
             const double i_z = wave_scan_f64(zi, lane), i_q = wave_scan_f64(qi, lane);
             if (j <= ncs) {
                 const uint32_t e_n = c_n + (i_n - n);
                 const double e_z = c_z + (i_z - zi), e_q = c_q + (i_q - qi);
-                const float e_c = (float)(c_c + (i_c - ci)) * (1.0f / 256.0f) - (float)e_n;
-                const float e_s = (float)(c_s + (i_s - si)) * (1.0f / 256.0f) - (float)e_n;
                 LocalEdge e;
                 e.q = e_n;
                 e.zm = (float)(e_z * (1.0 / 32768.0) - 8.0 * (double)e_n);
                 e.sq = (float)(e_q * (1.0 / 8192.0));
-                e.cs = local_edge_trig(e_c, e_s);
+                e.cs = 0u;
+                if (!FLAT) {
+                    const float e_c = (float)(c_c + (i_c - ci)) * (1.0f / 256.0f) - (float)e_n;
+                    const float e_s = (float)(c_s + (i_s - si)) * (1.0f / 256.0f) - (float)e_n;
+                    e.cs = local_edge_trig(e_c, e_s);
+                }
                 out[(size_t)ra * (ncs + 1u) + j] = e;
             }
             c_n += (uint32_t)__builtin_amdgcn_readlane((int)i_n, 63);
-            c_c += (uint32_t)__builtin_amdgcn_readlane((int)i_c, 63);
-            c_s += (uint32_t)__builtin_amdgcn_readlane((int)i_s, 63);
+            if (!FLAT) {
+                c_c += (uint32_t)__builtin_amdgcn_readlane((int)i_c, 63);
+                c_s += (uint32_t)__builtin_amdgcn_readlane((int)i_s, 63);
+            }
             c_z += lane_value(i_z, 63);
             c_q += lane_value(i_q, 63);
         }
     }
-    for (int off = 32; off >= 1; off >>= 1) {
-        zlo = fminf(zlo, __shfl_xor(zlo, off, 64));
-        zhi = fmaxf(zhi, __shfl_xor(zhi, off, 64));
-        flag |= (uint32_t)__shfl_xor((int)flag, off, 64);
-    }
-    if (lane == 0u) { l_zlo[wave] = zlo; l_zhi[wave] = zhi; l_flag[wave] = flag; }
+    for (int off = 32; off >= 1; off >>= 1) flag |= (uint32_t)__shfl_xor((int)flag, off, 64);
+    if (lane == 0u) l_flag[wave] = flag;
     __syncthreads();
     if (tid == 0u) {
-        for (uint32_t w = 1; w < 16u; w++) { zlo = fminf(zlo, l_zlo[w]); zhi = fmaxf(zhi, l_zhi[w]); flag |= l_flag[w]; }
-        reinterpret_cast<uint4 *>(a.finfo)[s] = zlo <= zhi ? make_uint4(local_float_key(zlo), local_float_key(zhi), flag & 1u, 2u)
-                                                            : make_uint4(0xffffffffu, 0u, flag & 1u, 2u);
+        for (uint32_t w = 1; w < 16u; w++) flag |= l_flag[w];
+        const uint32_t made = FLAT ? 6u : 2u;
+        reinterpret_cast<uint4 *>(a.finfo)[s] = zlo <= zhi ? make_uint4(local_float_key(zlo), local_float_key(zhi), flag & 1u, made)
+                                                            : make_uint4(0xffffffffu, 0u, flag & 1u, made);
         if (flag) { a.need[s] = 1u; a.need[a.n_slab] = 1u; }
+        if (FLAT) atomicAdd(&a.sums_stats[0], 1u);
     }
 }
 
@@ -1831,6 +1880,8 @@
     uint32_t nca, ncb, ka, kb, ncs, n_rows;
     int da, db, dn;
     float La, Lb, Ln, z_min, z_max;
+    bool flat;
+    float flat_g, flat_eps, flat_tan, flat_kq;
 };
 template <typename EdgePtr>
 __device__ __forceinline__ bool local_decide_head(const LocalArgs &a, const DecideFrame &F, uint32_t f, uint32_t m, EdgePtr edge,
@@ -1856,7 +1907,7 @@
     const float r_in = thr * (1.0f - 4e-4f), r_out = thr * (1.0f + 4e-4f);
     const float inv_cb = __builtin_amdgcn_rcpf(cb), t0 = fb * inv_cb + (float)kb, two_kb = (float)(2u * kb);
     uint32_t c_n = 0, r_n = 0;
-    float c_z = 0.0f, r_z = 0.0f, r_q = 0.0f, c_c = 0.0f, c_s = 0.0f;
+    float c_z = 0.0f, r_z = 0.0f, r_q = 0.0f, c_c = 0.0f, c_s = 0.0f, i_q = 0.0f;
     bool spans_ok = true;
     for (uint32_t sub0 = 0; sub0 < n_rows; sub0 += 4u) {
         LocalEdge e_a[4], e_d[4], e_lo[4], e_hi[4];
@@ -1896,10 +1947,14 @@
             r_n += n_c - (e_hi[u].q - e_lo[u].q);
             r_z += z_c - (e_hi[u].zm - e_lo[u].zm);
             r_q += (e_d[u].sq - e_a[u].sq) - (e_hi[u].sq - e_lo[u].sq);
-            float dc, ds;
-            local_edge_trig_diff(e_d[u].cs, e_a[u].cs, dc, ds);
-            c_c += dc;
-            c_s += ds;
+            if (F.flat) {
+                i_q += e_hi[u].sq - e_lo[u].sq;
+            } else {
+                float dc, ds;
+                local_edge_trig_diff(e_d[u].cs, e_a[u].cs, dc, ds);
+                c_c += dc;
+                c_s += ds;
+            }
             spans_ok &= n_c < kEdgeSpanMax;
         }
     }
@@ -1908,13 +1963,17 @@
     const float B = __builtin_fmaxf((r_q - 2.0f * hm * r_z) + fr * hm * hm, 0.0f) * 1.02f + 1e-3f * fr;
     const float mid = T - 0.5f * A, rad = 0.5005f * __builtin_amdgcn_sqrtf(fr * B);
     const float slack = 0.1f + fn * (1.05e-3f + 1e-6f * fn * Ln);
-    const float r_c = __builtin_amdgcn_sqrtf(c_c * c_c + c_s * c_s);
-    const float est_c = (local_atan2_fast(-c_s, -c_c) + 3.1415927f) * (Ln * 0.15915494f);
-    const float shift_c = gm_min_image(hn_pos - est_c, Ln, bad);
-    const float e_c = fr + 1.0f + 0.004f * fn;
-    const float xr = e_c * __builtin_amdgcn_rcpf(r_c);
-    const float emargin = 1e-4f * Ln + (xr + 0.5708f * xr * xr * xr) * (0.15916f * Ln);
-    const bool same_image = e_c < r_c && ulo_g + shift_c > -halfn + emargin && uhi_g + shift_c < halfn - emargin;
+    const float z_i = c_z - r_z, q_i = __builtin_fmaxf((i_q - 2.0f * F.flat_g * z_i) + fi * F.flat_g * F.flat_g, 0.0f);
+    bool same_image = (fi - F.flat_kq * q_i) - fr * F.flat_eps > fn * F.flat_tan + 1.0f;
+    if (!F.flat) {
+        const float r_c = __builtin_amdgcn_sqrtf(c_c * c_c + c_s * c_s);
+        const float est_c = (local_atan2_fast(-c_s, -c_c) + 3.1415927f) * (Ln * 0.15915494f);
+        const float shift_c = gm_min_image(hn_pos - est_c, Ln, bad);
+        const float e_c = fr + 1.0f + 0.004f * fn;
+        const float xr = e_c * __builtin_amdgcn_rcpf(r_c);
+        const float emargin = 1e-4f * Ln + (xr + 0.5708f * xr * xr * xr) * (0.15916f * Ln);
+        same_image = e_c < r_c && ulo_g + shift_c > -halfn + emargin && uhi_g + shift_c < halfn - emargin;
+    }
     const bool head_near = __builtin_fabsf(mid) + rad < (halfn - 1e-3f * Ln) * fi;
     centre_above = mid > 0.0f;
     return !redo && spans_ok && c_n > r_n && same_image && head_near && a.prune != 2 &&
@@ -1950,6 +2009,14 @@
     F.da = (int)((a.dim + 1u) % 3u); F.db = (int)((a.dim + 2u) % 3u); F.dn = (int)a.dim;
     F.La = box[F.da]; F.Lb = box[F.db]; F.Ln = box[F.dn];
     F.z_min = local_key_float(fk.x); F.z_max = local_key_float(fk.y);
+    F.flat = (fk.w & 4u) != 0u;
+    {
+        const float eps = __builtin_fmaxf(3.1415927f * (F.z_max - F.z_min) / F.Ln - 1.5707963f, 0.0f) + 0.01f;
+        F.flat_g = 0.5f * (F.z_min + F.z_max) - 0.5f * F.Ln;
+        F.flat_eps = eps;
+        F.flat_tan = 1.05f * (eps + eps * eps * eps) + 0.02f;
+        F.flat_kq = 19.739209f / (F.Ln * F.Ln);
+    }
     const bool fail = !(F.ka >= 1u && F.kb >= 1u && F.n_rows <= 16u && fk.z == 0u && fk.x <= fk.y);
     if (a.sums && s == 0u && threadIdx.x == 0u) a.todo[0] = make_uint2(0u, 0u);
     if (fail || !(F.z_max - F.z_min < 0.75f * F.Ln) || (int)s == a.write_dist_frame || (a.sums && a.need[s] != 0u)) {
diff --git a/include/gorder_hip.h b/include/gorder_hip.h
--- a/include/gorder_hip.h
+++ b/include/gorder_hip.h
@@ -240,6 +240,8 @@
 
 int gorder_hip_local_decide_stats(gorder_hip_handle *h, uint64_t out[4]);
 
+int gorder_hip_local_sums_stats(gorder_hip_handle *h, uint64_t out[4]);
+
 int gorder_hip_selftest_arithmetic(int device, uint64_t n, uint64_t seed, uint64_t mismatches[2]);
 int gorder_hip_selftest_trig(int device, int fn, uint32_t first_bits, uint32_t stride, uint32_t n, float *out);
 
```
